# borgwang/tinynn-autograd

Measured on NVIDIA B200. Metric: MLP train samples/sec, higher is better.
Workload: dtype f32 (tensor-core GEMMs: 3-term split on scaled fp16 hi/lo planes, fp32 accumulate)

## Files before the change

### core/_backend.py

```python
import ctypes
import gc
import os
import weakref

import numpy as np

_HERE = os.path.dirname(os.path.abspath(__file__))
_ROOT = os.path.dirname(_HERE)
LIB_PATH = os.environ.get(
    "TNN_B200_LIB", os.path.join(_ROOT, "tinynn-autograd_b200", "libtnn_b200.so"))

F32 = np.dtype(np.float32)
F64 = np.dtype(np.float64)
_DT_CODE = {F32: 0, F64: 1}
MAX_DIMS = 8

ADD, SUB, MUL, DIV, POW, MAXIMUM, MINIMUM, GE, GT, LE, LT, EQ = range(12)
MUL_GE, MUL_GT, MUL_LE, MUL_LT, MUL_EQ, DIV_BWD_B, POW_BWD_A, POW_BWD_B = range(20, 28)
NEG, EXP, LOG, COPY, CLIP, SCALE, CLIP_BWD, RECIP_MUL = range(40, 48)
RED_SUM, RED_MAX, RED_MIN = 0, 1, 2
OPT_SGD, OPT_ADAM, OPT_RMSPROP, OPT_MOMENTUM, OPT_ADAGRAD, OPT_ADADELTA = range(6)

_c_i64 = ctypes.c_int64
_c_i32 = ctypes.c_int32
_c_int = ctypes.c_int
_c_vp = ctypes.c_void_p
_c_dbl = ctypes.c_double
_c_sz = ctypes.c_size_t

_lib = None
_inited = False


class BackendError(RuntimeError):
    pass


_SIGNATURES = {
    "tnn_init": [_c_int],
    "tnn_shutdown": [],
    "tnn_sync": [],
    "tnn_device_info": [_c_vp, _c_vp, _c_vp, _c_vp, _c_vp],
    "tnn_device_count": [_c_vp],
    "tnn_alloc": [_c_sz, _c_vp],
    "tnn_free": [_c_vp],
    "tnn_pool_stats": [_c_vp, _c_vp, _c_vp],
    "tnn_pool_trim": [],
    "tnn_h2d": [_c_vp, _c_vp, _c_sz],
    "tnn_d2h": [_c_vp, _c_vp, _c_sz],
    "tnn_d2d": [_c_vp, _c_vp, _c_sz],
    "tnn_memset": [_c_vp, _c_int, _c_sz],
    "tnn_host_alloc": [_c_sz, _c_vp],
    "tnn_host_free": [_c_vp],
    "tnn_host_register": [_c_vp, _c_sz],
    "tnn_host_unregister": [_c_vp],
    "tnn_h2d_async_copy_stream": [_c_vp, _c_vp, _c_sz],
    "tnn_copy_stream_sync": [],
    "tnn_copy_wait_compute": [],
    "tnn_compute_wait_copy": [],
    "tnn_event_create": [_c_vp],
    "tnn_event_destroy": [_c_vp],
    "tnn_event_record": [_c_vp],
    "tnn_event_elapsed_ms": [_c_vp, _c_vp, _c_vp],
    "tnn_prof_enable": [_c_int],
    "tnn_prof_collect": [_c_vp, _c_vp],
    "tnn_l2_flush": [],
    "tnn_graph_begin": [],
    "tnn_graph_end": [_c_vp],
    "tnn_graph_abort": [],
    "tnn_graph_launch": [_c_vp],
    "tnn_graph_info": [_c_vp, _c_vp, _c_vp, _c_vp],
    "tnn_graph_destroy": [_c_vp],
    "tnn_ew": [_c_int, _c_int, _c_vp, _c_vp, _c_vp, _c_vp, _c_int, _c_vp, _c_vp, _c_vp, _c_vp,
               _c_dbl, _c_dbl, _c_int],
    "tnn_ew_flat": [_c_int, _c_int, _c_vp, _c_vp, _c_vp, _c_vp, _c_i64, _c_int, _c_dbl, _c_dbl,
                    _c_int],
    "tnn_cast": [_c_int, _c_vp, _c_int, _c_vp, _c_i64],
    "tnn_fill": [_c_int, _c_vp, _c_dbl, _c_i64],
    "tnn_reduce": [_c_int, _c_int, _c_vp, _c_vp, _c_i64, _c_i64, _c_i64],
    "tnn_unbroadcast": [_c_int, _c_vp, _c_vp, _c_int, _c_vp, _c_vp],
    "tnn_strided_copy": [_c_int, _c_vp, _c_vp, _c_int, _c_vp, _c_vp, _c_vp],
    "tnn_gather_rows": [_c_int, _c_vp, _c_vp, _c_vp, _c_i64, _c_i64, _c_i64],
    "tnn_scatter_rows": [_c_int, _c_vp, _c_vp, _c_vp, _c_i64, _c_i64, _c_i64],
    "tnn_gather_flat": [_c_int, _c_vp, _c_vp, _c_vp, _c_i64],
    "tnn_scatter_flat": [_c_int, _c_vp, _c_vp, _c_vp, _c_i64],
    "tnn_gemm_simt": [_c_int, _c_vp, _c_i64, _c_vp, _c_i64, _c_i64, _c_vp, _c_i64, _c_i64, _c_i64,
                      _c_i64, _c_i64, _c_vp, _c_int, _c_vp, _c_vp],
    "tnn_dense_bwd_simt": [_c_int, _c_vp, _c_vp, _c_vp, _c_vp, _c_vp, _c_vp, _c_vp, _c_int, _c_vp, _c_int,
                           _c_i64, _c_i64, _c_i64],
    "tnn_split_tf32": [_c_vp, _c_i64, _c_i64, _c_vp, _c_vp, _c_i64, _c_vp, _c_vp, _c_i64],
    "tnn_gemm_tf32x3": [_c_vp, _c_i64, _c_vp, _c_vp, _c_i64, _c_vp, _c_vp, _c_i64, _c_i64, _c_i64,
                        _c_i64, _c_vp, _c_int, _c_int, _c_vp, _c_vp, _c_vp, _c_i64, _c_vp],
    "tnn_split_tf32_bf16": [_c_vp, _c_i64, _c_i64, _c_vp, _c_vp, _c_vp, _c_i64],
    "tnn_gemm_tf32_bf16x2": [_c_vp, _c_i64, _c_vp, _c_vp, _c_vp, _c_i64, _c_vp, _c_vp, _c_vp, _c_i64,
                             _c_i64, _c_i64, _c_i64, _c_vp, _c_int, _c_int, _c_vp, _c_vp, _c_vp, _c_vp,
                             _c_i64, _c_vp],
    "tnn_f16_stats": [_c_vp, _c_i64, _c_vp, _c_int],
    "tnn_set_gemm_f16_cluster": [_c_int],
    "tnn_f16_meta_reset": [_c_vp],
    "tnn_split_f16": [_c_vp, _c_i64, _c_i64, _c_vp, _c_vp, _c_i64, _c_vp, _c_int],
    "tnn_gemm_f16x3": [_c_vp, _c_i64, _c_vp, _c_vp, _c_i64, _c_vp, _c_vp, _c_vp, _c_i64, _c_vp, _c_i64,
                       _c_i64, _c_i64, _c_vp, _c_int, _c_int, _c_vp, _c_vp, _c_vp],
    "tnn_split_tf32_bf16_cond": [_c_vp, _c_i64, _c_i64, _c_vp, _c_vp, _c_vp, _c_i64, _c_int,
                                 _c_vp, _c_i64, _c_i64, _c_vp, _c_vp, _c_vp, _c_i64, _c_int, _c_vp, _c_vp, _c_vp],
    "tnn_f16_stats_cond": [_c_vp, _c_i64, _c_vp, _c_int],
    "tnn_gemm_tf32_bf16x2_cond": [_c_vp, _c_i64, _c_vp, _c_vp, _c_vp, _c_i64, _c_vp, _c_vp, _c_vp, _c_i64,
                                  _c_i64, _c_i64, _c_i64, _c_vp, _c_int, _c_int, _c_vp, _c_vp, _c_vp, _c_vp],
    "tnn_set_gemm_cta_group": [_c_int],
    "tnn_set_gemm_ksplit": [_c_int],
    "tnn_set_gemm_group_m": [_c_int],
    "tnn_relu_fwd": [_c_int, _c_vp, _c_vp, _c_i64],
    "tnn_relu_bwd": [_c_int, _c_vp, _c_vp, _c_vp, _c_i64],
    "tnn_colsum": [_c_int, _c_vp, _c_vp, _c_i64, _c_i64],
    "tnn_ce_stats": [_c_int, _c_vp, _c_i64, _c_i64, _c_vp],
    "tnn_ce_merge_stats": [_c_int, _c_vp, _c_vp, _c_int],
    "tnn_ce_loss": [_c_int, _c_vp, _c_int, _c_vp, _c_i64, _c_i64, _c_vp, _c_dbl, _c_vp, _c_vp, _c_vp],
    "tnn_ce_fwd_small": [_c_int, _c_vp, _c_int, _c_vp, _c_i64, _c_i64, _c_dbl, _c_vp, _c_vp, _c_vp, _c_vp],
    "tnn_ce_bwd": [_c_int, _c_vp, _c_vp, _c_int, _c_vp, _c_i64, _c_i64, _c_vp, _c_vp, _c_dbl, _c_vp, _c_vp,
                   _c_vp],
    "tnn_set_gemm_reserved_sms": [_c_int],
    "tnn_d2h_async": [_c_vp, _c_vp, _c_sz, _c_vp],
    "tnn_event_sync": [_c_vp],
    "tnn_one_hot": [_c_int, _c_vp, _c_vp, _c_i64, _c_i64],
    "tnn_mlp_tail_workspace": [_c_int, _c_vp, _c_vp, _c_i64, _c_vp, _c_vp, _c_vp],
    "tnn_mlp_tail_step": [_c_int, _c_vp, _c_vp, _c_vp, _c_vp, _c_vp, _c_vp, _c_i64, _c_vp, _c_vp, _c_int,
                          _c_i64, _c_dbl, _c_vp, _c_vp, _c_vp, _c_vp, _c_vp, _c_vp, _c_vp],
    "tnn_opt_step": [_c_int, _c_int, _c_vp, _c_vp, _c_vp, _c_vp, _c_vp, _c_i64, _c_vp, _c_int],
    "tnn_opt_step_dev": [_c_int, _c_int, _c_vp, _c_vp, _c_vp, _c_vp, _c_vp, _c_i64, _c_vp],
    "tnn_nccl_unique_id": [_c_vp],
    "tnn_nccl_init": [_c_int, _c_int, _c_vp],
    "tnn_nccl_destroy": [],
    "tnn_allreduce_sum": [_c_int, _c_vp, _c_i64],
    "tnn_allgather": [_c_int, _c_vp, _c_vp, _c_i64],
    "tnn_comm_wait_compute": [],
    "tnn_compute_wait_comm": [],
    "tnn_allreduce_sum_comm": [_c_int, _c_vp, _c_i64],
    "tnn_nccl_version": [_c_vp],
}
EXPORTED_SYMBOLS = sorted(list(_SIGNATURES) + ["tnn_last_error", "tnn_stream", "tnn_launch_count",
                                                "tnn_alloc_ptr"])


def load_library():
    global _lib
    if _lib is not None:
        return _lib
    if not os.path.exists(LIB_PATH):
        raise BackendError(
            "libtnn_b200.so not found at %s -- build it with `python tinynn-autograd_b200/build.py` "
            "(there is no CPU fallback)" % LIB_PATH)
    lib = ctypes.CDLL(LIB_PATH)
    for name, argtypes in _SIGNATURES.items():
        fn = getattr(lib, name)
        fn.argtypes = argtypes
        fn.restype = _c_int
    lib.tnn_last_error.argtypes = []
    lib.tnn_last_error.restype = ctypes.c_char_p
    lib.tnn_stream.argtypes = []
    lib.tnn_stream.restype = _c_vp
    lib.tnn_launch_count.argtypes = []
    lib.tnn_launch_count.restype = ctypes.c_uint64
    lib.tnn_alloc_ptr.argtypes = [_c_sz]
    lib.tnn_alloc_ptr.restype = _c_vp
    _lib = lib
    return lib


def _raise(name):
    msg = _lib.tnn_last_error().decode("utf-8", "replace")
    raise BackendError("%s failed: %s" % (name, msg))


def init(device=None):
    global _inited
    if _inited:
        return
    lib = load_library()
    if device is None:
        device = int(os.environ.get("TNN_DEVICE", os.environ.get("LOCAL_RANK", "0")))
    if lib.tnn_init(int(device)):
        _raise("tnn_init")
    _inited = True


def is_initialized():
    return _inited


def sync():
    init()
    if _lib.tnn_sync():
        _raise("tnn_sync")


def launch_count():
    return int(_lib.tnn_launch_count()) if _lib is not None else 0


def device_info():
    init()
    sm, maj, mnr = _c_int(), _c_int(), _c_int()
    tot, l2 = _c_sz(), _c_sz()
    if _lib.tnn_device_info(ctypes.byref(sm), ctypes.byref(maj), ctypes.byref(mnr),
                            ctypes.byref(tot), ctypes.byref(l2)):
        _raise("tnn_device_info")
    return {"sm_count": sm.value, "cc": (maj.value, mnr.value), "total_mem": tot.value,
            "l2_bytes": l2.value}


def set_gemm_reserved_sms(n):
    init()
    if _lib.tnn_set_gemm_reserved_sms(int(n)):
        _raise("tnn_set_gemm_reserved_sms")


def pool_stats():
    a, b, c = _c_sz(), _c_sz(), _c_sz()
    _lib.tnn_pool_stats(ctypes.byref(a), ctypes.byref(b), ctypes.byref(c))
    return {"reserved": a.value, "in_use": b.value, "cuda_mallocs": c.value}


_SMALL_MAX = 1 << 20
_SMALL_KEEP = 64
_SMALL_CAP_BYTES = 256 << 20
_small_free = {}
_small_bytes = 0
_capturing = False


class _Buf(object):
    __slots__ = ("ptr", "nbytes", "klass", "__weakref__")

    def __init__(self, nbytes):
        self.nbytes = nbytes
        if nbytes <= _SMALL_MAX and not _capturing:
            klass = (nbytes + 511) & ~511
            lst = _small_free.get(klass)
            if lst:
                global _small_bytes
                _small_bytes -= klass
                self.ptr = lst.pop()
                self.klass = klass
                return
            nbytes = klass
            self.klass = klass
        else:
            self.klass = 0
        ptr = _lib.tnn_alloc_ptr(nbytes)
        if not ptr:
            self.ptr = None
            _raise("tnn_alloc")
        self.ptr = ptr

    def __del__(self):
        try:
# ... 184 lines not shown
    arr = np.asarray(arr)
    dt = device_dtype(arr.dtype if dtype is None else dtype)
    host = np.require(arr, dtype=dt, requirements="C")
    out = empty(host.shape, dt)
    if host.size:
        if _lib.tnn_h2d(out.ptr, host.ctypes.data, host.nbytes):
            _raise("tnn_h2d")
    return out


def upload_into(dst, host):
    host = np.require(host, dtype=dst.dtype, requirements="C")
    assert host.size == dst.size
    if host.size and _lib.tnn_h2d(dst.ptr, host.ctypes.data, host.nbytes):
        _raise("tnn_h2d")


def to_numpy(d):
    out = np.empty(d.shape, dtype=d.dtype)
    if d.size:
        if _lib.tnn_d2h(out.ctypes.data, d.ptr, out.nbytes):
            _raise("tnn_d2h")
    return out


def full(shape, value, dtype):
    out = empty(shape, dtype)
    if out.size:
        if _lib.tnn_fill(_DT_CODE[out.dtype], out.ptr, float(value), out.size):
            _raise("tnn_fill")
    return out


_ONES = {}


def ones_scalar(dtype):
    dtype = np.dtype(dtype)
    one = _ONES.get(dtype)
    if one is None:
        one = _ONES[dtype] = full((), 1.0, dtype)
    return one


def zeros(shape, dtype):
    out = empty(shape, dtype)
    if out.size:
        if _lib.tnn_memset(out.ptr, 0, out.nbytes):
            _raise("tnn_memset")
    return out


def memset_zero(d):
    if d.size and _lib.tnn_memset(d.ptr, 0, d.nbytes):
        _raise("tnn_memset")


def copy_into(dst, src):
    assert dst.size == src.size and dst.dtype == src.dtype
    if dst.size and _lib.tnn_d2d(dst.ptr, src.ptr, dst.nbytes):
        _raise("tnn_d2d")


def clone(d):
    out = empty(d.shape, d.dtype)
    copy_into(out, d)
    return out


def astype(d, dtype):
    dtype = np.dtype(dtype)
    if d.dtype == dtype:
        return d
    out = empty(d.shape, dtype)
    if d.size and _lib.tnn_cast(_DT_CODE[dtype], out.ptr, _DT_CODE[d.dtype], d.ptr, d.size):
        _raise("tnn_cast")
    return out


def upload_index(idx):
    idx = np.ascontiguousarray(idx, dtype=np.int64)
    out = empty(idx.shape, F64)
    if idx.size and _lib.tnn_h2d(out.ptr, idx.ctypes.data, idx.nbytes):
        _raise("tnn_h2d")
    return out


def _i64arr(vals):
    return (_c_i64 * len(vals))(*vals)


def _bstrides(shape, out_shape):
    nd = len(out_shape)
    pad = nd - len(shape)
    st = [0] * nd
    acc = 1
    for i in range(len(shape) - 1, -1, -1):
        if shape[i] != 1:
            st[pad + i] = acc
        acc *= shape[i]
    return st


def _common_dtype(*arrs):
    for a in arrs:
        if a.dtype == F64:
            return F64
    return F32


def ew(op, x, y=None, z=None, p0=0.0, p1=0.0, flags=0, out=None):
    ops_ = [a for a in (x, y, z) if a is not None]
    dt = _common_dtype(*ops_)
    ops_ = [a if a.dtype == dt else astype(a, dt) for a in ops_]
    if len(ops_) == 1:
        oshape = ops_[0].shape
    else:
        oshape = ops_[0].shape
        for a in ops_[1:]:
            if a.shape != oshape:
                oshape = np.broadcast_shapes(*[a.shape for a in ops_])
                break
    if out is None:
        out = empty(oshape, dt)
    n = out.size
    if n == 0:
        return out
    ptrs = [a.ptr for a in ops_] + [None] * (3 - len(ops_))
    mask = 0
    flat = True
    for i, a in enumerate(ops_):
        if a.size == 1:
            mask |= 1 << i
        elif a.shape != oshape:
            if a.size == n and _bstrides(a.shape, oshape) == _bstrides(oshape, oshape):
                continue
            flat = False
    if flat:
        if _lib.tnn_ew_flat(op, _DT_CODE[dt], out.ptr, ptrs[0], ptrs[1], ptrs[2], n, mask,
                            p0, p1, flags):
            _raise("tnn_ew_flat")
        return out
    nd = len(oshape)
    if nd > MAX_DIMS:
        raise ValueError("tensors of rank > %d are not supported" % MAX_DIMS)
    st = [_i64arr(_bstrides(a.shape, oshape)) for a in ops_] + [None] * (3 - len(ops_))
    if _lib.tnn_ew(op, _DT_CODE[dt], out.ptr, ptrs[0], ptrs[1], ptrs[2], nd, _i64arr(oshape),
                   st[0], st[1], st[2], p0, p1, flags):
        _raise("tnn_ew")
    return out


def add_inplace(dst, src):
    if src.dtype != dst.dtype:
        src = astype(src, dst.dtype)
    if _lib.tnn_ew_flat(ADD, _DT_CODE[dst.dtype], dst.ptr, dst.ptr, src.ptr, None, dst.size,
                        2 if (src.size == 1 and dst.size != 1) else 0, 0.0, 0.0, 0):
        _raise("tnn_ew_flat")
    return dst


def broadcast_to(d, shape):
    shape = tuple(shape)
    if d.shape == shape:
        return d
    out = empty(shape, d.dtype)
    oshape = np.broadcast_shapes(d.shape, shape)
    if tuple(oshape) != shape:
        raise ValueError("cannot broadcast %s to %s" % (d.shape, shape))
    if out.size:
        if _lib.tnn_ew(COPY, _DT_CODE[d.dtype], out.ptr, d.ptr, None, None, len(shape),
                       _i64arr(shape), _i64arr(_bstrides(d.shape, shape)), None, None, 0.0, 0.0, 0):
            _raise("tnn_ew")
    return out


def reduce(red_op, x, axis=None):
    if axis is None:
        outer, red, inner = 1, x.size, 1
        oshape = ()
    else:
        nd = x.ndim
        if not -nd <= axis < nd:
            raise np.exceptions.AxisError(axis, nd)
        axis %= nd
        outer = _prod(x.shape[:axis])
        red = x.shape[axis]
        inner = _prod(x.shape[axis + 1:])
        oshape = x.shape[:axis] + x.shape[axis + 1:]
    if red == 0 and red_op != RED_SUM:
        raise ValueError("zero-size array to reduction operation which has no identity")
    out = empty(oshape, x.dtype)
    if out.size:
        if _lib.tnn_reduce(red_op, _DT_CODE[x.dtype], out.ptr, x.ptr, outer, red, inner):
            _raise("tnn_reduce")
    return out


def unbroadcast(g, shape):
    shape = tuple(shape)
    if g.shape == shape:
        return g
    nd = g.ndim
    lead = nd - len(shape)
    if lead < 0:
        raise ValueError("gradient of rank %d for a tensor of rank %d" % (nd, len(shape)))
    keep = [0] * lead + [0 if s == 1 else 1 for s in shape]
    for i in range(len(shape)):
        if shape[i] != 1 and shape[i] != g.shape[lead + i]:
            raise ValueError("operands could not be broadcast together with shapes %s %s"
                             % (g.shape, shape))
    out = empty(shape, g.dtype)
    if out.size:
        if _lib.tnn_unbroadcast(_DT_CODE[g.dtype], out.ptr, g.ptr, nd, _i64arr(g.shape),
                                (_c_i32 * nd)(*keep)):
            _raise("tnn_unbroadcast")
    return out


def colsum(g, out=None):
    R, C = g.shape
    if out is None:
        out = empty((1, C), g.dtype)
    if _lib.tnn_colsum(_DT_CODE[g.dtype], out.ptr, g.ptr, R, C):
        _raise("tnn_colsum")
    return out


def _cstrides(shape):
    st = [0] * len(shape)
    acc = 1
    for i in range(len(shape) - 1, -1, -1):
        st[i] = acc
        acc *= shape[i]
    return st


def permute(x, axes):
    nd = x.ndim
    axes = [a % nd for a in axes]
    oshape = tuple(x.shape[a] for a in axes)
    out = empty(oshape, x.dtype)
    if out.size:
        xs = _cstrides(x.shape)
        if _lib.tnn_strided_copy(_DT_CODE[x.dtype], out.ptr, x.ptr, nd, _i64arr(oshape),
                                 _i64arr(_cstrides(oshape)), _i64arr([xs[a] for a in axes])):
            _raise("tnn_strided_copy")
    return out


def strided_copy(dst, dst_off, dst_strides, src, src_off, src_strides, shape):
    if _prod(shape) == 0:
        return
    isz = dst.dtype.itemsize
    if _lib.tnn_strided_copy(_DT_CODE[dst.dtype], dst.ptr + dst_off * isz, src.ptr + src_off * isz,
                             len(shape), _i64arr(shape), _i64arr(dst_strides), _i64arr(src_strides)):
        _raise("tnn_strided_copy")


def one_hot_into(out, labels_i32_ptr, n_rows, n_classes):
    if _lib.tnn_one_hot(_DT_CODE[out.dtype], out.ptr, labels_i32_ptr, n_rows, n_classes):
        _raise("tnn_one_hot")


def gather_rows(x, idx_dev, n_idx):
    row = _prod(x.shape[1:])
    out = empty((n_idx,) + x.shape[1:], x.dtype)
    if out.size and _lib.tnn_gather_rows(_DT_CODE[x.dtype], out.ptr, x.ptr, idx_dev.ptr, n_idx, row,
                                         x.shape[0]):
        _raise("tnn_gather_rows")
    return out


def scatter_rows(g, idx_dev, n_idx, shape):
    out = zeros(shape, g.dtype)
    row = _prod(shape[1:])
    if g.size and _lib.tnn_scatter_rows(_DT_CODE[g.dtype], out.ptr, g.ptr, idx_dev.ptr, n_idx, row,
                                        shape[0]):
        _raise("tnn_scatter_rows")
    return out


def gather_flat(x, idx_dev, oshape):
    out = empty(oshape, x.dtype)
    if out.size and _lib.tnn_gather_flat(_DT_CODE[x.dtype], out.ptr, x.ptr, idx_dev.ptr, out.size):
        _raise("tnn_gather_flat")
    return out


def scatter_flat(g, idx_dev, shape):
    out = zeros(shape, g.dtype)
    if g.size and _lib.tnn_scatter_flat(_DT_CODE[g.dtype], out.ptr, g.ptr, idx_dev.ptr, g.size):
        _raise("tnn_scatter_flat")
    return out


TC_MIN_MNK = int(os.environ.get("TNN_TC_MIN_MNK", str(1 << 29)))
TC_ENABLED = os.environ.get("TNN_TC", "1") != "0"
TC_MN_MAJOR = os.environ.get("TNN_TC_MN_MAJOR", "1") != "0"
TC_SPLIT = os.environ.get("TNN_GEMM_SPLIT", "f16")
LAZY_RELU_OUT = os.environ.get("TNN_LAZY_RELU", "1") != "0"
BF16_BYTES = 2
_split_epoch = 0


def new_split_epoch():
    global _split_epoch
    _split_epoch += 1


def _round4(n):
    return (n + 3) // 4 * 4


def _round8(n):
    return (n + 7) // 8 * 8


def _empty_16bit(rows, ld):
    return empty((rows, ld // 2), F32)


def split_planes_mix(x):
    cache = x.split
    if cache is None or cache.get("epoch") != _split_epoch:
        cache = {"epoch": _split_epoch}
        x.split = cache
    if "m" in cache:
        return cache["m"]
    R, C = x.shape
    ld = _round8(C)
    hi, h16, l16 = empty((R, ld), F32), _empty_16bit(R, ld), _empty_16bit(R, ld)
    if _lib.tnn_split_tf32_bf16(x.ptr, R, C, hi.ptr, h16.ptr, l16.ptr, ld):
        _raise("tnn_split_tf32_bf16")
    cache["m"] = (hi, h16, l16, ld)
    return cache["m"]


F16_PITCH_PAD = int(os.environ.get("TNN_F16_PITCH_PAD", "0"))


def _new_meta():
    return empty((8,), F32)


def split_planes_f16(x):
    cache = x.split
    if cache is None or cache.get("epoch") != _split_epoch:
        cache = {"epoch": _split_epoch}
        x.split = cache
    if "f" in cache:
        return cache["f"]
    R, C = x.shape
    ld = _round8(C) + F16_PITCH_PAD
    if type(x) is LazyReLU and x._real is None:
        src, relu_mode = x._src, 1
    else:
        src, relu_mode = x, 0
    meta = cache.get("stat")
    if meta is None:
        meta = _new_meta()
        if _lib.tnn_f16_stats(src.ptr, R * C, meta.ptr, relu_mode):
            _raise("tnn_f16_stats")
    elif _lib.tnn_f16_stats_cond(src.ptr, R * C, meta.ptr, relu_mode):
        _raise("tnn_f16_stats_cond")
    hf, l16 = _empty_16bit(R, ld), _empty_16bit(R, ld)
    if _lib.tnn_split_f16(src.ptr, R, C, hf.ptr, l16.ptr, ld, meta.ptr, relu_mode):
        _raise("tnn_split_f16")
    cache["f"] = (hf, l16, ld, meta, src if src is not x else None, relu_mode)
    return cache["f"]


_FALLBACK_PLANES = {}
_FALLBACK_CAP_BYTES = 16 << 30
_fallback_bytes = 0


def _fallback_planes(role, R, ld):
    if _capturing:
        return (empty((R, ld), F32), _empty_16bit(R, ld), _empty_16bit(R, ld))
    global _fallback_bytes
    key = (role, R, ld)
    p = _FALLBACK_PLANES.get(key)
    if p is None:
        if _fallback_bytes > _FALLBACK_CAP_BYTES:
            sync()
            _FALLBACK_PLANES.clear()
            _fallback_bytes = 0
        p = (empty((R, ld), F32), _empty_16bit(R, ld), _empty_16bit(R, ld))
        _FALLBACK_PLANES[key] = p
        _fallback_bytes += 8 * R * ld
    return p


def _matmul_f16(a, b, ta, tb, bias, out, flags, act, mask_src, M, N, K):
    a_hf, a_l16, lda, a_meta, a_src, a_relu = split_planes_f16(a)
    b_hf, b_l16, ldb, b_meta, b_src, b_relu = split_planes_f16(b)
    a_src = a if a_src is None else a_src
    b_src = b if b_src is None else b_src
    layout = (1 if ta else 0) | (0 if tb else 2)
    act_out = None
    stat = None
    if act:
        stat = _new_meta()
        if _lib.tnn_f16_meta_reset(stat.ptr):
            _raise("tnn_f16_meta_reset")
        if mask_src is None and LAZY_RELU_OUT:
            act_out = LazyReLU(out)
            flags |= 8
        else:
            act_out = empty((M, N), F32)
    real_act = act_out if (act and type(act_out) is not LazyReLU) else None
    bias_p = bias.ptr if bias is not None else None
    mask_p = mask_src.ptr if (act and mask_src is not None) else None
    if _lib.tnn_gemm_f16x3(out.ptr, N, a_hf.ptr, a_l16.ptr, lda, a_meta.ptr, b_hf.ptr, b_l16.ptr, ldb,
                           b_meta.ptr, M, N, K, bias_p, flags, layout,
                           real_act.ptr if real_act is not None else None, mask_p,
                           stat.ptr if stat is not None else None):
        _raise("tnn_gemm_f16x3")
    fa = _fallback_planes(0, a.shape[0], lda)
    fb = _fallback_planes(1, b.shape[0], ldb)
    if _lib.tnn_split_tf32_bf16_cond(a_src.ptr, a.shape[0], a.shape[1], fa[0].ptr, fa[1].ptr, fa[2].ptr, lda,
                                     a_relu, b_src.ptr, b.shape[0], b.shape[1], fb[0].ptr, fb[1].ptr,
                                     fb[2].ptr, ldb, b_relu, a_meta.ptr, b_meta.ptr,
                                     stat.ptr if stat is not None else None):
        _raise("tnn_split_tf32_bf16_cond")
    if _lib.tnn_gemm_tf32_bf16x2_cond(out.ptr, N, fa[0].ptr, fa[1].ptr, fa[2].ptr, lda, fb[0].ptr, fb[1].ptr,
                                      fb[2].ptr, ldb, M, N, K, bias_p, flags & 3, layout,
                                      real_act.ptr if real_act is not None else None, mask_p,
                                      a_meta.ptr, b_meta.ptr):
        _raise("tnn_gemm_tf32_bf16x2_cond")
    if act:
        act_out.split = {"epoch": _split_epoch, "stat": stat}
        return out, act_out
    return out


def split_planes(x, transposed, also_other=False):
    cache = x.split
    if cache is None or cache.get("epoch") != _split_epoch:
        cache = {"epoch": _split_epoch}
        x.split = cache
    key = "t" if transposed else "p"
    if key in cache:
        return cache[key]
    R, C = x.shape
    want_p = (not transposed) or (also_other and "p" not in cache)
    want_t = transposed or (also_other and "t" not in cache)
    hi = lo = hit = lot = None
    ldp = _round4(C)
    ldt = _round4(R)
    if want_p:
        hi, lo = empty((R, ldp), F32), empty((R, ldp), F32)
    if want_t:
        hit, lot = empty((C, ldt), F32), empty((C, ldt), F32)
    if _lib.tnn_split_tf32(x.ptr, R, C, hi.ptr if hi else None, lo.ptr if lo else None, ldp,
                           hit.ptr if hit else None, lot.ptr if lot else None, ldt):
        _raise("tnn_split_tf32")
    if want_p:
        cache["p"] = (hi, lo, ldp)
    if want_t:
        cache["t"] = (hit, lot, ldt)
    return cache[key]


def set_gemm_cta_group(cg):
    load_library()
    if _lib.tnn_set_gemm_cta_group(int(cg)):
        _raise("tnn_set_gemm_cta_group")


def set_gemm_f16_cluster(cl):
    load_library()
    if _lib.tnn_set_gemm_f16_cluster(int(cl)):
        _raise("tnn_set_gemm_f16_cluster")


def set_gemm_ksplit(ks):
    load_library()
    if _lib.tnn_set_gemm_ksplit(int(ks)):
        _raise("tnn_set_gemm_ksplit")


def use_tensor_cores(M, N, K, dtype):
    return (TC_ENABLED and dtype == F32 and M >= 64 and N >= 64 and K >= 32
            and M * N * K >= TC_MIN_MNK)


def matmul(a, b, ta=False, tb=False, bias=None, out=None, accumulate=False, relu=False,
           reuse_a=False, reuse_b=False, act=False, mask_src=None):
    if a.ndim != 2 or b.ndim != 2:
        raise ValueError("matmul: only 2-D operands are supported (got %s @ %s)" % (a.shape, b.shape))
    dt = _common_dtype(a, b)
    if a.dtype != dt:
        a = astype(a, dt)
    if b.dtype != dt:
        b = astype(b, dt)
    M, K = (a.shape[1], a.shape[0]) if ta else a.shape
    K2, N = (b.shape[1], b.shape[0]) if tb else b.shape
    if K != K2:
        raise ValueError("matmul: shapes %s and %s not aligned" % ((M, K), (K2, N)))
    if out is None:
        out = empty((M, N), dt)
        accumulate = False
    elif out.dtype != dt or out.shape != (M, N):
        raise ValueError("matmul: bad output array")
    if bias is not None and bias.dtype != dt:
        bias = astype(bias, dt)
    act_out = empty((M, N), dt) if act else None
    if M == 0 or N == 0:
        return (out, act_out) if act else out
    flags = (1 if accumulate else 0) | (2 if relu else 0)
    if K > 0 and use_tensor_cores(M, N, K, dt) and TC_SPLIT == "f16":
        return _matmul_f16(a, b, ta, tb, bias, out, flags, act, mask_src, M, N, K)
    if K > 0 and use_tensor_cores(M, N, K, dt) and TC_SPLIT == "mix":
        a_hi, a_h16, a_l16, lda = split_planes_mix(a)
        b_hi, b_h16, b_l16, ldb = split_planes_mix(b)
        layout = (1 if ta else 0) | (0 if tb else 2)
        act_hi = act_h16 = act_l16 = None
        ld_act = _round8(N)
        if act:
            act_hi = empty((M, ld_act), F32)
            act_h16, act_l16 = _empty_16bit(M, ld_act), _empty_16bit(M, ld_act)
            if LAZY_RELU_OUT and mask_src is None:
                act_out = LazyReLU(out)
        if _lib.tnn_gemm_tf32_bf16x2(out.ptr, N, a_hi.ptr, a_h16.ptr, a_l16.ptr, lda, b_hi.ptr,
                                     b_h16.ptr, b_l16.ptr, ldb, M, N, K,
                                     bias.ptr if bias is not None else None, flags, layout,
                                     act_out.ptr if (act and type(act_out) is not LazyReLU) else None,
                                     act_hi.ptr if act else None,
                                     act_h16.ptr if act else None, act_l16.ptr if act else None,
                                     ld_act, mask_src.ptr if (act and mask_src is not None) else None):
            _raise("tnn_gemm_tf32_bf16x2")
        if act:
            act_out.split = {"epoch": _split_epoch, "m": (act_hi, act_h16, act_l16, ld_act)}
            return out, act_out
        return out
    if K > 0 and use_tensor_cores(M, N, K, dt):
        if TC_MN_MAJOR:
            a_hi, a_lo, lda = split_planes(a, transposed=False)
            b_hi, b_lo, ldb = split_planes(b, transposed=False)
            layout = (1 if ta else 0) | (0 if tb else 2)
        else:
            a_hi, a_lo, lda = split_planes(a, transposed=ta, also_other=reuse_a)
            b_hi, b_lo, ldb = split_planes(b, transposed=not tb, also_other=reuse_b)
            layout = 0
        act_hi = act_lo = None
        ld_act = _round4(N)
        if act:
            act_hi, act_lo = empty((M, ld_act), F32), empty((M, ld_act), F32)
        if _lib.tnn_gemm_tf32x3(out.ptr, N, a_hi.ptr, a_lo.ptr, lda, b_hi.ptr, b_lo.ptr, ldb, M, N,
                                K, bias.ptr if bias is not None else None, flags, layout,
                                act_out.ptr if act else None, act_hi.ptr if act else None,
                                act_lo.ptr if act else None, ld_act,
                                mask_src.ptr if (act and mask_src is not None) else None):
            _raise("tnn_gemm_tf32x3")
        if act:
            act_out.split = {"epoch": _split_epoch, "p": (act_hi, act_lo, ld_act)}
            return out, act_out
        return out
    a_rs, a_cs = (1, a.shape[1]) if ta else (a.shape[1], 1)
    b_rs, b_cs = (1, b.shape[1]) if tb else (b.shape[1], 1)
    if mask_src is not None and mask_src.dtype != dt:
        mask_src = astype(mask_src, dt)
    if _lib.tnn_gemm_simt(_DT_CODE[dt], out.ptr, N, a.ptr, a_rs, a_cs, b.ptr, b_rs, b_cs, M, N, K,
                          bias.ptr if bias is not None else None, flags & 1,
                          act_out.ptr if act else None,
                          mask_src.ptr if (act and mask_src is not None) else None):
        _raise("tnn_gemm_simt")
    if relu:
        if _lib.tnn_relu_fwd(_DT_CODE[dt], out.ptr, out.ptr, out.size):
            _raise("tnn_relu_fwd")
    return (out, act_out) if act else out


GROUPED_BWD_MAX_TILES = 1024


def dense_bwd_grouped_ok(B, K, N, dtype):
    if use_tensor_cores(B, K, N, dtype) or use_tensor_cores(K, N, B, dtype):
        return False
    t = lambda m, n: ((m + 31) // 32) * ((n + 31) // 32)
    return t(K, N) + t(B, K) + t(1, N) <= GROUPED_BWD_MAX_TILES


def dense_bwd_grouped(g, x, w, mask_src, need_dx, dw_out, dw_acc, db_out, db_acc):
    B, N = g.shape
    K = w.shape[0]
    dx = empty((B, K), g.dtype) if need_dx else None
    masked = empty((B, K), g.dtype) if (need_dx and mask_src is not None) else None
    if _lib.tnn_dense_bwd_simt(_DT_CODE[g.dtype], g.ptr, x.ptr, w.ptr,
                               mask_src.ptr if masked is not None else None,
                               dx.ptr if dx is not None else None,
                               masked.ptr if masked is not None else None,
                               dw_out.ptr, 1 if dw_acc else 0, db_out.ptr, 1 if db_acc else 0, B, K, N):
        _raise("tnn_dense_bwd_simt")
    return dx, masked


def relu_fwd(x):
    out = empty(x.shape, x.dtype)
    if x.size and _lib.tnn_relu_fwd(_DT_CODE[x.dtype], out.ptr, x.ptr, x.size):
        _raise("tnn_relu_fwd")
    return out


def relu_bwd(g, x):
    if g.dtype != x.dtype:
        g = astype(g, x.dtype)
    out = empty(x.shape, x.dtype)
    if x.size and _lib.tnn_relu_bwd(_DT_CODE[x.dtype], out.ptr, g.ptr, x.ptr, x.size):
        _raise("tnn_relu_bwd")
    return out


def ce_stats(z):
    B, C = z.shape
    stats = empty((2,), z.dtype)
    if _lib.tnn_ce_stats(_DT_CODE[z.dtype], z.ptr, B, C, stats.ptr):
        _raise("tnn_ce_stats")
    return stats


def ce_merge_stats(stats_all, n_ranks):
    out = empty((2,), stats_all.dtype)
    if _lib.tnn_ce_merge_stats(_DT_CODE[stats_all.dtype], out.ptr, stats_all.ptr, n_ranks):
        _raise("tnn_ce_merge_stats")
    return out


def _ce_labels(y):
    if type(y) is LazyOneHot and y._real is None:
        return None, y.labels_ptr
    return y.ptr, None


def ce_loss(z, y, stats, m_global):
    B, C = z.shape
    q = empty((B,), z.dtype)
    loss = empty((), z.dtype)
    y_ptr, lab_ptr = _ce_labels(y)
    if _lib.tnn_ce_loss(_DT_CODE[z.dtype], z.ptr, _DT_CODE[y.dtype], y_ptr, B, C, stats.ptr,
                        float(m_global), q.ptr, loss.ptr, lab_ptr):
        _raise("tnn_ce_loss")
    return loss, q


def ce_small_ok(B, C):
    return B <= 2048 and B * C <= 16384


def ce_fwd_small(z, y, m_global, want_dz=False):
    B, C = z.shape
    stats, q, loss = empty((2,), z.dtype), empty((B,), z.dtype), empty((), z.dtype)
    dz = empty((B, C), z.dtype) if want_dz else None
    if _lib.tnn_ce_fwd_small(_DT_CODE[z.dtype], z.ptr, _DT_CODE[y.dtype], y.ptr, B, C,
                             float(m_global), stats.ptr, q.ptr, loss.ptr, dz.ptr if want_dz else None):
        _raise("tnn_ce_fwd_small")
    return stats, loss, q, dz


def is_ones_scalar(g):
    one = _ONES.get(np.dtype(g.dtype))
    return one is not None and g is one


def ce_bwd(z, y, stats, q, m_global, g):
    B, C = z.shape
    dz = empty((B, C), z.dtype)
    if g.dtype != z.dtype:
        g = astype(g, z.dtype)
    stat = None
    if z.dtype == F32 and TC_SPLIT == "f16" and TC_ENABLED and B * C >= (1 << 16):
        stat = _new_meta()
        if _lib.tnn_f16_meta_reset(stat.ptr):
            _raise("tnn_f16_meta_reset")
    y_ptr, lab_ptr = _ce_labels(y)
    if _lib.tnn_ce_bwd(_DT_CODE[z.dtype], dz.ptr, z.ptr, _DT_CODE[y.dtype], y_ptr, B, C, stats.ptr,
                       q.ptr, float(m_global), g.ptr, stat.ptr if stat is not None else None, lab_ptr):
        _raise("tnn_ce_bwd")
    if stat is not None:
        dz.split = {"epoch": _split_epoch, "stat": stat}
    return dz


class MLPTail(object):

    MAX_WIDTH = 256
    MAX_LAYERS = 6
    SMEM_LIMIT = 220 * 1024

    def __init__(self, dims, batch, n_grad):
        L = len(dims) - 1
        self.L, self.batch, self.n_grad = L, batch, n_grad
        self.in_dims = (_c_i64 * L)(*dims[:-1])
        self.out_dims = (_c_i64 * L)(*dims[1:])
        smem, n_ctas, scratch = _c_i64(), _c_i64(), _c_i64()
        if _lib.tnn_mlp_tail_workspace(L, self.in_dims, self.out_dims, batch, ctypes.byref(smem),
                                       ctypes.byref(n_ctas), ctypes.byref(scratch)):
            _raise("tnn_mlp_tail_workspace")
        self.smem_bytes, self.n_ctas = smem.value, n_ctas.value
        self.scratch = empty((scratch.value,), F32)
        self.stats = zeros((2 * self.n_ctas,), F32)
        self.loss_part = zeros((self.n_ctas,), F32)
        self.counters = zeros((16,), F32)
        self.logits = empty((batch, dims[-1]), F32)
        self.dlogits = self.scratch.view((batch, dims[-1]), scratch.value - batch * dims[-1])

    @classmethod
    def eligible(cls, dims, batch):
        init()
        L = len(dims) - 1
        if not (1 <= L <= cls.MAX_LAYERS) or any(d < 1 or d > cls.MAX_WIDTH for d in dims):
            return False
        if batch < 1 or batch > 256:
            return False
        floats = sum(dims[i] * (dims[i + 1] | 1) + (dims[i + 1] + 3) // 4 * 4 for i in range(L))
        floats = (floats + 3) // 4 * 4 + 12 * sum(dims) + 4 * 256
        return floats * 4 <= cls.SMEM_LIMIT

    def run(self, ws, bs, grad_base, grad_offsets, n_grad, z1, y, m_global, dz1, loss_out):
        if n_grad != self.n_grad:
            raise ValueError("MLPTail was laid out for %d gradient elements, got %d" % (self.n_grad, n_grad))
        wp = (_c_vp * self.L)(*[w.ptr for w in ws])
        bp = (_c_vp * self.L)(*[b.ptr for b in bs])
        go = (_c_i64 * (2 * self.L))(*grad_offsets)
        if _lib.tnn_mlp_tail_step(self.L, self.in_dims, self.out_dims, wp, bp, go, grad_base.ptr, n_grad,
                                  z1.ptr, y.ptr, _DT_CODE[y.dtype], self.batch, float(m_global), dz1.ptr,
                                  loss_out.ptr, self.scratch.ptr, self.stats.ptr, self.loss_part.ptr,
                                  self.counters.ptr, self.logits.ptr):
            _raise("tnn_mlp_tail_step")


def opt_step(opt, param, step_out, grad, s0, s1, hyper):
    n = grad.size
    if isinstance(hyper, DArray):
        if _lib.tnn_opt_step_dev(opt, _DT_CODE[grad.dtype], param.ptr if param is not None else None,
                                 step_out.ptr if step_out is not None else None, grad.ptr,
                                 s0.ptr if s0 is not None else None,
                                 s1.ptr if s1 is not None else None, n, hyper.ptr):
            _raise("tnn_opt_step_dev")
        return
    h = (_c_dbl * len(hyper))(*hyper)
    if _lib.tnn_opt_step(opt, _DT_CODE[grad.dtype], param.ptr if param is not None else None,
                         step_out.ptr if step_out is not None else None, grad.ptr,
                         s0.ptr if s0 is not None else None, s1.ptr if s1 is not None else None,
                         n, h, len(hyper)):
        _raise("tnn_opt_step")


class PinnedArray(object):

    def __init__(self, shape, dtype):
        init()
        self.shape = tuple(shape)
        self.dtype = np.dtype(dtype)
        nbytes = max(_prod(self.shape), 1) * self.dtype.itemsize
        p = _c_vp()
        if _lib.tnn_host_alloc(nbytes, ctypes.byref(p)):
            _raise("tnn_host_alloc")
        self.ptr = p.value
        self.nbytes = nbytes
        raw = (ctypes.c_char * nbytes).from_address(self.ptr)
        self.array = np.frombuffer(raw, dtype=self.dtype, count=_prod(self.shape)).reshape(self.shape)

    def __del__(self):
        try:
            if self.ptr and _lib is not None:
                self.array = None
                _lib.tnn_host_free(self.ptr)
                self.ptr = None
        except Exception:
            pass


class RegisteredHostArray(object):

    def __init__(self, array):
        init()
        if not (isinstance(array, np.ndarray) and array.flags["C_CONTIGUOUS"]):
            raise ValueError("only C-contiguous numpy arrays can be pinned in place")
        self.array = array
        self.ptr = array.ctypes.data
        if _lib.tnn_host_register(self.ptr, array.nbytes):
            _raise("tnn_host_register")

    def row_address(self, row):
        return self.ptr + row * self.array.strides[0]

    def __del__(self):
        try:
            if self.ptr and _lib is not None:
                _lib.tnn_host_unregister(self.ptr)
                self.ptr = None
        except Exception:
            pass


def h2d_prefetch(dst, pinned):
    if _lib.tnn_copy_wait_compute():
        _raise("tnn_copy_wait_compute")
    src = pinned if isinstance(pinned, int) else pinned.ptr
    if _lib.tnn_h2d_async_copy_stream(dst.ptr, src, dst.nbytes):
        _raise("tnn_h2d_async_copy_stream")


def copy_stream_sync():
    if _lib.tnn_copy_stream_sync():
        _raise("tnn_copy_stream_sync")


def wait_prefetch():
    if _lib.tnn_compute_wait_copy():
        _raise("tnn_compute_wait_copy")


_pinned_free = {}


class AsyncRead(object):

    def __init__(self, d):
        init()
        self.shape, self.dtype = d.shape, d.dtype
        nbytes = max(d.nbytes, 1)
        free = _pinned_free.get(nbytes)
        self.pin = free.pop() if free else PinnedArray((nbytes,), np.uint8)
        self.event = Event()
        self._src = d
        self._value = None
        if _lib.tnn_d2h_async(self.pin.ptr, d.ptr, d.nbytes, self.event.ptr):
            _raise("tnn_d2h_async")

    def result(self):
        if self._value is None:
# ... 130 lines not shown
```

### include/tnn_b200.h

```cpp
#ifndef TNN_B200_H
#define TNN_B200_H

#include <stddef.h>
#include <stdint.h>

#ifdef __cplusplus
extern "C" {
#endif

#define TNN_MAX_DIMS 8
#define TNN_F32 0
#define TNN_F64 1

enum {
  TNN_OP_ADD = 0,
  TNN_OP_SUB = 1,
  TNN_OP_MUL = 2,
  TNN_OP_DIV = 3,
  TNN_OP_POW = 4,
  TNN_OP_MAXIMUM = 5,
  TNN_OP_MINIMUM = 6,
  TNN_OP_GE = 7,
  TNN_OP_GT = 8,
  TNN_OP_LE = 9,
  TNN_OP_LT = 10,
  TNN_OP_EQ = 11,
  TNN_OP_MUL_GE = 20,
  TNN_OP_MUL_GT = 21,
  TNN_OP_MUL_LE = 22,
  TNN_OP_MUL_LT = 23,
  TNN_OP_MUL_EQ = 24,
  TNN_OP_DIV_BWD_B = 25,
  TNN_OP_POW_BWD_A = 26,
  TNN_OP_POW_BWD_B = 27,
  TNN_OP_NEG = 40,
  TNN_OP_EXP = 41,
  TNN_OP_LOG = 42,
  TNN_OP_COPY = 43,
  TNN_OP_CLIP = 44,
  TNN_OP_SCALE = 45,
  TNN_OP_CLIP_BWD = 46,
  TNN_OP_RECIP_MUL = 47
};

enum { TNN_RED_SUM = 0, TNN_RED_MAX = 1, TNN_RED_MIN = 2 };

enum {
  TNN_OPT_SGD = 0,
  TNN_OPT_ADAM = 1,
  TNN_OPT_RMSPROP = 2,
  TNN_OPT_MOMENTUM = 3,
  TNN_OPT_ADAGRAD = 4,
  TNN_OPT_ADADELTA = 5
};

const char* tnn_last_error(void);
int tnn_init(int device);
int tnn_shutdown(void);
int tnn_sync(void);
int tnn_device_info(int* sm_count, int* cc_major, int* cc_minor, size_t* total_mem, size_t* l2_bytes);
int tnn_device_count(int* n);
void* tnn_stream(void);
uint64_t tnn_launch_count(void);

int tnn_alloc(size_t nbytes, void** out);
void* tnn_alloc_ptr(size_t nbytes);
int tnn_free(void* p);
int tnn_pool_stats(size_t* reserved_bytes, size_t* in_use_bytes, size_t* n_cuda_malloc);
int tnn_pool_trim(void);
int tnn_h2d(void* dst, const void* src, size_t nbytes);
int tnn_d2h(void* dst, const void* src, size_t nbytes);
int tnn_d2h_async(void* pinned_dst, const void* src, size_t nbytes, void* done_event);
int tnn_event_sync(void* ev);
int tnn_d2d(void* dst, const void* src, size_t nbytes);
int tnn_memset(void* dst, int byte, size_t nbytes);
int tnn_host_alloc(size_t nbytes, void** out);
int tnn_host_free(void* p);
int tnn_host_register(void* p, size_t nbytes);
int tnn_host_unregister(void* p);
int tnn_h2d_async_copy_stream(void* dst, const void* pinned_src, size_t nbytes);
int tnn_copy_stream_sync(void);
int tnn_copy_wait_compute(void);
int tnn_compute_wait_copy(void);
int tnn_event_create(void** ev);
int tnn_event_destroy(void* ev);
int tnn_event_record(void* ev);
int tnn_event_elapsed_ms(void* start, void* stop, float* ms);
int tnn_prof_enable(int family);
int tnn_prof_collect(double* total_ms, uint64_t* n_launches);
int tnn_l2_flush(void);

int tnn_graph_begin(void);
int tnn_graph_end(void** graph_out);
int tnn_graph_abort(void);
int tnn_graph_launch(void* graph);
int tnn_graph_info(void* graph, size_t* n_nodes, size_t* n_kernel_nodes, size_t* n_blocks);
int tnn_graph_destroy(void* graph);

int tnn_ew(int op, int dtype, void* out, const void* x, const void* y, const void* z,
           int ndim, const int64_t* shape,
           const int64_t* xs, const int64_t* ys, const int64_t* zs,
           double p0, double p1, int flags);
int tnn_ew_flat(int op, int dtype, void* out, const void* x, const void* y, const void* z,
                int64_t n, int scalar_mask, double p0, double p1, int flags);
int tnn_cast(int dst_dtype, void* dst, int src_dtype, const void* src, int64_t n);
int tnn_fill(int dtype, void* dst, double value, int64_t n);

int tnn_reduce(int red_op, int dtype, void* out, const void* x,
               int64_t outer, int64_t red, int64_t inner);
int tnn_unbroadcast(int dtype, void* out, const void* grad, int ndim,
                    const int64_t* gshape, const int32_t* keep);

int tnn_strided_copy(int dtype, void* dst, const void* src, int ndim, const int64_t* shape,
                     const int64_t* dst_strides, const int64_t* src_strides);
int tnn_gather_rows(int dtype, void* out, const void* x, const int64_t* idx_dev,
                    int64_t n_idx, int64_t row_elems, int64_t n_rows_src);
int tnn_scatter_rows(int dtype, void* out, const void* g, const int64_t* idx_dev,
                     int64_t n_idx, int64_t row_elems, int64_t n_rows_dst);
int tnn_gather_flat(int dtype, void* out, const void* x, const int64_t* idx_dev, int64_t n);
int tnn_scatter_flat(int dtype, void* out, const void* g, const int64_t* idx_dev, int64_t n);
int tnn_one_hot(int dtype, void* out, const int32_t* labels_dev, int64_t B, int64_t C);

int tnn_gemm_simt(int dtype, void* C, int64_t ldc, const void* A, int64_t a_rs, int64_t a_cs,
                  const void* B, int64_t b_rs, int64_t b_cs, int64_t M, int64_t N, int64_t K,
                  const void* bias, int flags, void* act_out, const void* mask_src);
int tnn_dense_bwd_simt(int dtype, const void* g, const void* x, const void* w, const void* mask_src,
                       void* dx, void* dx_masked, void* dw, int dw_accumulate, void* db,
                       int db_accumulate, int64_t B, int64_t K, int64_t N);
int tnn_split_tf32(const float* x, int64_t R, int64_t C,
                   float* hi, float* lo, int64_t ldp, float* hiT, float* loT, int64_t ldt);
int tnn_gemm_tf32x3(float* D, int64_t ldd,
                    const float* a_hi, const float* a_lo, int64_t lda,
                    const float* b_hi, const float* b_lo, int64_t ldb,
                    int64_t M, int64_t N, int64_t K, const float* bias, int flags, int layout,
                    float* act_out, float* act_hi, float* act_lo, int64_t ld_act,
                    const float* mask_src);
int tnn_split_tf32_bf16(const float* x, int64_t R, int64_t C, float* hi, void* h16, void* l16,
                        int64_t ld);
int tnn_gemm_tf32_bf16x2(float* D, int64_t ldd,
                         const float* a_hi, const void* a_h16, const void* a_l16, int64_t lda,
                         const float* b_hi, const void* b_h16, const void* b_l16, int64_t ldb,
                         int64_t M, int64_t N, int64_t K, const float* bias, int flags, int layout,
                         float* act_out, float* act_hi, void* act_h16, void* act_l16, int64_t ld_act,
                         const float* mask_src);
int tnn_f16_stats(const float* x, int64_t n, void* meta, int relu_mode);
int tnn_set_gemm_f16_cluster(int cl);
int tnn_f16_meta_reset(void* meta);
int tnn_split_f16(const float* x, int64_t R, int64_t C, void* hf, void* l16, int64_t ld, void* meta,
                  int relu_mode);
int tnn_gemm_f16x3(float* D, int64_t ldd, const void* a_hf, const void* a_l16, int64_t lda,
                   const void* a_meta, const void* b_hf, const void* b_l16, int64_t ldb,
                   const void* b_meta, int64_t M, int64_t N, int64_t K, const float* bias, int flags,
                   int layout, float* act_out, const float* mask_src, void* stat_meta);
int tnn_split_tf32_bf16_cond(const float* xa, int64_t Ra, int64_t Ca, float* hia, void* h16a, void* l16a,
                             int64_t lda, int relu_a, const float* xb, int64_t Rb, int64_t Cb, float* hib,
                             void* h16b, void* l16b, int64_t ldb, int relu_b, const void* meta_a,
                             const void* meta_b, void* result_meta);
int tnn_f16_stats_cond(const float* x, int64_t n, void* meta, int relu_mode);
int tnn_gemm_tf32_bf16x2_cond(float* D, int64_t ldd, const float* a_hi, const void* a_h16,
                              const void* a_l16, int64_t lda, const float* b_hi, const void* b_h16,
                              const void* b_l16, int64_t ldb, int64_t M, int64_t N, int64_t K,
                              const float* bias, int flags, int layout, float* act_out,
                              const float* mask_src, const void* meta_a, const void* meta_b);
int tnn_set_gemm_cta_group(int cg);
int tnn_set_gemm_reserved_sms(int n);
int tnn_set_gemm_ksplit(int ks);
int tnn_set_gemm_group_m(int gm);

int tnn_relu_fwd(int dtype, void* out, const void* x, int64_t n);
int tnn_relu_bwd(int dtype, void* dx, const void* g, const void* x, int64_t n);
int tnn_colsum(int dtype, void* out, const void* g, int64_t R, int64_t C);

int tnn_ce_stats(int dtype, const void* z, int64_t B, int64_t C, void* stats_dev);
int tnn_ce_merge_stats(int dtype, void* stats_out_dev, const void* stats_all_dev, int n_ranks);
int tnn_ce_loss(int dtype, const void* z, int y_dtype, const void* y, int64_t B, int64_t C,
                const void* stats_dev, double m_global, void* q_dev, void* loss_dev,
                const int32_t* labels_dev);
int tnn_ce_fwd_small(int dtype, const void* z, int y_dtype, const void* y, int64_t B, int64_t C,
                     double m_global, void* stats_dev, void* q_dev, void* loss_dev,
                     void* dz_dev );
int tnn_ce_bwd(int dtype, void* dz, const void* z, int y_dtype, const void* y, int64_t B, int64_t C,
               const void* stats_dev, const void* q_dev, double m_global, const void* g_dev,
               void* stat_meta ,
               const int32_t* labels_dev);

int tnn_mlp_tail_workspace(int n_layers, const int64_t* in_dims, const int64_t* out_dims, int64_t batch,
                           int64_t* smem_bytes, int64_t* n_ctas, int64_t* scratch_floats);
int tnn_mlp_tail_step(int n_layers, const int64_t* in_dims, const int64_t* out_dims, const void* const* w,
                      const void* const* b, const int64_t* grad_off, void* grad, int64_t n_grad,
                      const void* z1, const void* y, int y_dtype, int64_t B, double m_global, void* dz1,
                      void* loss_out, void* scratch, void* stats, void* loss_part, void* counters,
                      void* logits_out );

int tnn_opt_step(int opt, int dtype, void* param, void* step_out, const void* grad, void* s0,
                 void* s1, int64_t n, const double* h, int n_h);
int tnn_opt_step_dev(int opt, int dtype, void* param, void* step_out, const void* grad, void* s0,
                     void* s1, int64_t n, const double* h_dev);

int tnn_nccl_unique_id(void* id128);
int tnn_nccl_init(int rank, int world, const void* id128);
int tnn_nccl_destroy(void);
int tnn_allreduce_sum(int dtype, void* buf, int64_t n);
int tnn_allgather(int dtype, void* recv, const void* send, int64_t n_per_rank);
int tnn_comm_wait_compute(void);
int tnn_compute_wait_comm(void);
int tnn_allreduce_sum_comm(int dtype, void* buf, int64_t n);
int tnn_nccl_version(int* v);

#ifdef __cplusplus
}
#endif
#endif
```

### tinynn-autograd_b200/build.py

```python
import concurrent.futures
import os
import shutil
import subprocess
import sys

HERE = os.path.dirname(os.path.abspath(__file__))
ROOT = os.path.dirname(HERE)
CSRC = os.path.join(HERE, "csrc")
OBJ = os.path.join(HERE, "build")
LIB = os.path.join(HERE, "libtnn_b200.so")

SOURCES = ["runtime.cu", "elementwise.cu", "reduce.cu", "layout.cu", "gemm_simt.cu",
           "gemm_tc.cu", "gemm_f16.cu", "fused.cu", "mlp_fused.cu", "comm.cu"]
HEADERS = [os.path.join(CSRC, "common.cuh"), os.path.join(CSRC, "math.cuh"), os.path.join(CSRC, "tc_ptx.cuh"),
           os.path.join(ROOT, "include", "tnn_b200.h")]

NVCC_FLAGS = ["-gencode", "arch=compute_100a,code=sm_100a", "-O3", "-lineinfo", "-std=c++17",
              "-Xcompiler", "-fPIC", "-diag-suppress", "550", "-split-compile", "0"]
NO_FMAD = {"elementwise.cu", "fused.cu", "reduce.cu"}


def _nvcc():
    return shutil.which("nvcc") or "/usr/local/cuda/bin/nvcc"


def _stale(target, deps):
    if not os.path.exists(target):
        return True
    t = os.path.getmtime(target)
    return any(os.path.getmtime(d) > t for d in deps)


def _compile(src, force):
    obj = os.path.join(OBJ, src.replace(".cu", ".o"))
    path = os.path.join(CSRC, src)
    if not force and not _stale(obj, [path] + HEADERS):
        return obj, False
    cmd = [_nvcc()] + NVCC_FLAGS + (["-fmad=false"] if src in NO_FMAD else []) + ["-c", path, "-o", obj]
    r = subprocess.run(cmd, capture_output=True, text=True)
    if r.returncode != 0:
        raise RuntimeError("nvcc failed for %s:\n%s\n%s" % (src, r.stdout[-4000:], r.stderr[-4000:]))
    return obj, True


def build(force=False, verbose=True):
    os.makedirs(OBJ, exist_ok=True)
    with concurrent.futures.ThreadPoolExecutor(max_workers=min(8, len(SOURCES))) as ex:
        results = list(ex.map(lambda s: _compile(s, force), SOURCES))
    objs = [o for o, _ in results]
    rebuilt = any(changed for _, changed in results)
    if rebuilt or _stale(LIB, objs):
        cmd = [_nvcc(), "-shared", "-o", LIB] + objs + ["-ldl"]
        r = subprocess.run(cmd, capture_output=True, text=True)
        if r.returncode != 0:
            raise RuntimeError("link failed:\n%s\n%s" % (r.stdout[-4000:], r.stderr[-4000:]))
        if verbose:
            print("built", LIB)
    elif verbose:
        print("up to date:", LIB)
    return LIB


if __name__ == "__main__":
    build(force="--force" in sys.argv)
```

### tinynn-autograd_b200/csrc/gemm_f16.cu

```cuda
#include <cuda.h>
#include <cuda_bf16.h>
#include <cuda_fp16.h>
#include <cudaTypedefs.h>

#include <algorithm>
#include <cstdlib>

#include "common.cuh"
#include "tc_ptx.cuh"

namespace tnn {
namespace tc {
extern int g_reserved_sms;
}
namespace f16 {

using namespace tnn::tc;

#ifndef TNN_F16_BK
#define TNN_F16_BK 64
#endif
#ifndef TNN_F16_STAGES
#define TNN_F16_STAGES (192 / TNN_F16_BK)
#endif
constexpr int BK = TNN_F16_BK;
constexpr int ROWS = 128;
constexpr int UMMA_N = 256;
constexpr int TILE_M = 256;
constexpr int UMMA_K = 16;
constexpr int PLANE_BYTES = ROWS * BK * 2;
constexpr int STAGE_BYTES = 4 * PLANE_BYTES;
constexpr int STAGES = TNN_F16_STAGES;
constexpr int CHUNK_KB = 256 / BK;
#ifndef TNN_F16_THREADS
#define TNN_F16_THREADS 384
#endif
constexpr int NUM_THREADS = TNN_F16_THREADS;
constexpr int EPI_WARP0 = NUM_THREADS == 320 ? 2 : 4;
constexpr uint32_t TMEM_COLS = 512;
constexpr int EPI_PATCH_BYTES = 8 * 4096;
constexpr int SMEM_BYTES = STAGES * STAGE_BYTES + 1024 + 256 + EPI_PATCH_BYTES;
#ifndef TNN_F16_KBOX_ROWS
#define TNN_F16_KBOX_ROWS 128
#endif
constexpr int KBOX_ROWS = TNN_F16_KBOX_ROWS;
constexpr int MN_BOX_BYTES = 64 * BK * 2;
constexpr float SMALL_LIMIT = 0.03125f;
constexpr unsigned int GUARD_FRACTION = 256;

struct Meta {
  unsigned int absmax;
  unsigned int need_stats;
  int exp;
  int safe;
  unsigned int n_small;
  unsigned int n_nz;
  unsigned int ticket;
  unsigned int pad;
};

__device__ __forceinline__ void meta_scale(unsigned int amax_bits, int& e, int& ok) {
  e = 0;
  ok = 1;
  if (amax_bits == 0u) return;
  if (amax_bits >= 0x7F800000u) { ok = 0; return; }
  const int ex = (int)(amax_bits >> 23) - 127;
  if (ex < -112) { ok = 0; return; }
  e = 14 - ex;
}

__device__ __forceinline__ float pow2f(int e) {
  return __int_as_float((e + 127) << 23);
}

template <bool MN>
__device__ __forceinline__ uint64_t make_desc(uint32_t saddr) {
  uint64_t d = 0;
  d |= (uint64_t)((saddr & 0x3FFFFu) >> 4);
  d |= (uint64_t)(MN ? (MN_BOX_BYTES >> 4) : 1) << 16;
  d |= (uint64_t)(((MN || BK == 64) ? 1024 : 512) >> 4) << 32;
  d |= (uint64_t)1 << 46;
  d |= (uint64_t)((MN || BK == 64) ? 2 : 4) << 61;
  return d;
}
__host__ __device__ constexpr uint32_t make_idesc(int a_fmt, int b_fmt, bool a_mn, bool b_mn) {
  return (1u << 4) | ((uint32_t)a_fmt << 7) | ((uint32_t)b_fmt << 10) | ((a_mn ? 1u : 0u) << 15) |
         ((b_mn ? 1u : 0u) << 16) | ((uint32_t)(UMMA_N >> 3) << 17) | ((uint32_t)(TILE_M >> 4) << 24);
}

__device__ __forceinline__ void tile_coords(int t, int tiles_m, int tiles_n, int group_m, int& tm, int& tn) {
  if (group_m == 1) {
    tm = t / tiles_n;
    tn = t - tm * tiles_n;
  } else if (group_m < 0) {
    const int gn = -group_m;
    const int per_panel = tiles_m * gn;
    const int g = t / per_panel;
    const int first_n = g * gn;
    const int cols = min(gn, tiles_n - first_n);
    const int r = t - g * per_panel;
    tm = r / cols;
    tn = first_n + r % cols;
  } else {
    const int per_group = group_m * tiles_n;
    const int g = t / per_group;
    const int first_m = g * group_m;
    const int rows = min(group_m, tiles_m - first_m);
    const int r = t - g * per_group;
    tm = first_m + r % rows;
    tn = r / rows;
  }
}

template <int CB>
__device__ __forceinline__ void patch_write(const float (&sum)[128], float4* patch, int lane, float f1,
                                            float f2, const float* bias_u, int colb, int N) {
#pragma unroll
  for (int c4 = 0; c4 < 8; ++c4) {
    float4 v = make_float4(sum[CB * 32 + c4 * 4] * f1 * f2, sum[CB * 32 + c4 * 4 + 1] * f1 * f2,
                           sum[CB * 32 + c4 * 4 + 2] * f1 * f2, sum[CB * 32 + c4 * 4 + 3] * f1 * f2);
    if (bias_u) {
      const int c = colb + c4 * 4;
      if (c + 3 < N) {
        const float4 b = *reinterpret_cast<const float4*>(bias_u + c);
        v.x += b.x; v.y += b.y; v.z += b.z; v.w += b.w;
      } else {
        if (c < N) v.x += bias_u[c];
        if (c + 1 < N) v.y += bias_u[c + 1];
        if (c + 2 < N) v.z += bias_u[c + 2];
      }
    }
    patch[lane * 8 + (c4 ^ (lane & 7))] = v;
  }
}

template <bool A_MN, bool B_MN, int CL>
__global__ void __launch_bounds__(NUM_THREADS, 1)
gemm_f16x3_kernel(const __grid_constant__ CUtensorMap map_a_h, const __grid_constant__ CUtensorMap map_a_l,
                  const __grid_constant__ CUtensorMap map_b_h, const __grid_constant__ CUtensorMap map_b_l,
                  float* __restrict__ D, int64_t ldd, int M, int N, int K,
                  const float* __restrict__ bias, int flags, int t_full, int tail_split,
                  unsigned int* __restrict__ tile_flags, float* __restrict__ act_out,
                  const float* __restrict__ mask_src, const Meta* __restrict__ meta_a,
                  const Meta* __restrict__ meta_b, Meta* __restrict__ stat_out, int group_m) {
  if (!(meta_a->safe && meta_b->safe)) return;
  extern __shared__ uint8_t smem_raw[];
  const uint32_t smem_base = (smem_u32(smem_raw) + 1023u) & ~1023u;
  uint8_t* smem_gen = smem_raw + (smem_base - smem_u32(smem_raw));
  const uint32_t bar_base = smem_base + STAGES * STAGE_BYTES;
  auto full_bar = [&](int s) { return bar_base + 8u * s; };
  auto empty_bar = [&](int s) { return bar_base + 8u * (STAGES + s); };
  auto tfull_bar = [&](int a) { return bar_base + 8u * (2 * STAGES + a); };
  auto tempty_bar = [&](int a) { return bar_base + 8u * (2 * STAGES + 2 + a); };
  const uint32_t tmem_ptr_smem = bar_base + 8u * (2 * STAGES + 4);
  volatile uint32_t* tmem_ptr_gen =
      reinterpret_cast<volatile uint32_t*>(smem_gen + STAGES * STAGE_BYTES + 8 * (2 * STAGES + 4));

  const int warp = threadIdx.x >> 5, lane = threadIdx.x & 31;
  const uint32_t cl_rank = cluster_ctarank();
  const uint32_t pair = cl_rank >> 1;
  const uint32_t cta_rank = cl_rank & 1u;
  const bool leader = cta_rank == 0;
  const uint16_t pair_mask = (uint16_t)(3u << (2 * pair));

  if (warp == 0 && lane == 0) {
    tma_prefetch_desc(&map_a_h);
    tma_prefetch_desc(&map_a_l);
    tma_prefetch_desc(&map_b_h);
    tma_prefetch_desc(&map_b_l);
    for (int s = 0; s < STAGES; ++s) {
      mbar_init(full_bar(s), 1);
      mbar_init(empty_bar(s), CL / 2);
    }
    for (int a = 0; a < 2; ++a) {
      mbar_init(tfull_bar(a), 1);
      mbar_init(tempty_bar(a), 16);
    }
    fence_barrier_init();
  }
  if (warp == 1) {
    tmem_alloc<2>(tmem_ptr_smem, TMEM_COLS);
    tmem_relinquish<2>();
  }
  tc_fence_before();
  cluster_sync_all();
  tc_fence_after();
  const uint32_t tmem_base = *tmem_ptr_gen;

  const int tiles_m = (M + TILE_M - 1) / TILE_M;
  const int tiles_n = (N + UMMA_N - 1) / UMMA_N;
  const int tiles_ns = CL == 4 ? (tiles_n + 1) / 2 : tiles_n;
  const int num_tiles = tiles_m * tiles_ns;
  const int num_kb = (K + BK - 1) / BK;
  const int group = blockIdx.x / CL;
  const int num_groups = gridDim.x / CL;
  const int tail_rem = num_tiles - t_full;
  const int num_units = t_full + tail_rem * tail_split;
  const int kb_per_split = (num_kb + tail_split - 1) / tail_split;
  auto decode = [&](int u, int& t, int& sp, int& kb_begin, int& kb_end) {
    if (u < t_full) {
      t = u; sp = 0; kb_begin = 0; kb_end = num_kb;
    } else {
      const int j = u - t_full;
      t = t_full + j % tail_rem;
      sp = j / tail_rem;
      kb_begin = sp * kb_per_split;
      kb_end = min(num_kb, kb_begin + kb_per_split);
    }
  };

  if (warp == 0) {
    if constexpr (NUM_THREADS == 384) asm volatile("setmaxnreg.dec.sync.aligned.u32 40;");
    if (lane == 0) {
      int stage = 0;
      uint32_t phase = 0;
      for (int u = group; u < num_units; u += num_groups) {
        int t, sp, kb_begin, kb_end;
        decode(u, t, sp, kb_begin, kb_end);
        int tm, tn;
        tile_coords((flags & 32) ? num_tiles - 1 - t : t, tiles_m, tiles_ns, group_m, tm, tn);
        if constexpr (CL == 4) tn = 2 * tn + (int)pair;
        const int row_a = tm * TILE_M + (int)cta_rank * ROWS;
        const int row_b = tn * UMMA_N + (int)cta_rank * ROWS;
        for (int kb = kb_begin; kb < kb_end; ++kb) {
          mbar_wait(empty_bar(stage), phase ^ 1u);
          const uint32_t sa_h = smem_base + stage * STAGE_BYTES;
          const uint32_t sa_l = sa_h + PLANE_BYTES;
          const uint32_t sb_h = sa_h + 2 * PLANE_BYTES;
          const uint32_t sb_l = sa_h + 3 * PLANE_BYTES;
          if (leader) mbar_expect_tx(full_bar(stage), (uint32_t)STAGE_BYTES * 2u);
          const int k0 = kb * BK;
          if (flags & 128) {
            if (leader)
              asm volatile("mbarrier.complete_tx.shared::cta.b64 [%0], %1;" ::"r"(full_bar(stage)), "r"((uint32_t)STAGE_BYTES * 2u) : "memory");
            if (++stage == STAGES) { stage = 0; phase ^= 1u; }
            continue;
          }
#ifdef TNN_F16_PREFETCH
          if (kb + TNN_F16_PREFETCH < kb_end) {
            const int kp = (kb + TNN_F16_PREFETCH) * BK;
            if constexpr (A_MN) {
#pragma unroll
              for (int j = 0; j < ROWS / 64; ++j) {
                tma_prefetch_l2_2d(&map_a_l, row_a + 64 * j, kp);
                tma_prefetch_l2_2d(&map_a_h, row_a + 64 * j, kp);
              }
            } else {
              tma_prefetch_l2_2d(&map_a_l, kp, row_a);
              tma_prefetch_l2_2d(&map_a_h, kp, row_a);
            }
            if constexpr (B_MN) {
#pragma unroll
              for (int j = 0; j < ROWS / 64; ++j) {
                tma_prefetch_l2_2d(&map_b_h, row_b + 64 * j, kp);
                tma_prefetch_l2_2d(&map_b_l, row_b + 64 * j, kp);
              }
            } else {
              tma_prefetch_l2_2d(&map_b_h, kp, row_b);
              tma_prefetch_l2_2d(&map_b_l, kp, row_b);
            }
          }
#endif
          if constexpr (CL == 4) {
            const uint16_t mc = (uint16_t)((1u << cta_rank) | (1u << (cta_rank + 2)));
            const uint32_t off = pair * (uint32_t)(PLANE_BYTES / 2);
            const int ra = row_a + 64 * (int)pair;
            if constexpr (A_MN) {
              tma_load_2d_pair_mc(sa_l + off, &map_a_l, full_bar(stage), ra, k0, mc);
              tma_load_2d_pair_mc(sa_h + off, &map_a_h, full_bar(stage), ra, k0, mc);
            } else {
              tma_load_2d_pair_mc(sa_l + off, &map_a_l, full_bar(stage), k0, ra, mc);
              tma_load_2d_pair_mc(sa_h + off, &map_a_h, full_bar(stage), k0, ra, mc);
            }
          } else if constexpr (A_MN) {
#pragma unroll
            for (int j = 0; j < ROWS / 64; ++j) {
              tma_load_2d<2>(sa_l + j * MN_BOX_BYTES, &map_a_l, full_bar(stage), row_a + 64 * j, k0);
              tma_load_2d<2>(sa_h + j * MN_BOX_BYTES, &map_a_h, full_bar(stage), row_a + 64 * j, k0);
            }
          } else {
#pragma unroll
            for (int j = 0; j < ROWS / KBOX_ROWS; ++j) {
              tma_load_2d<2>(sa_l + j * KBOX_ROWS * 128, &map_a_l, full_bar(stage), k0, row_a + j * KBOX_ROWS);
              tma_load_2d<2>(sa_h + j * KBOX_ROWS * 128, &map_a_h, full_bar(stage), k0, row_a + j * KBOX_ROWS);
            }
          }
          if constexpr (B_MN) {
#pragma unroll
            for (int j = 0; j < ROWS / 64; ++j) {
              tma_load_2d<2>(sb_h + j * MN_BOX_BYTES, &map_b_h, full_bar(stage), row_b + 64 * j, k0);
              tma_load_2d<2>(sb_l + j * MN_BOX_BYTES, &map_b_l, full_bar(stage), row_b + 64 * j, k0);
            }
          } else {
#pragma unroll
            for (int j = 0; j < ROWS / KBOX_ROWS; ++j) {
              tma_load_2d<2>(sb_h + j * KBOX_ROWS * 128, &map_b_h, full_bar(stage), k0, row_b + j * KBOX_ROWS);
              tma_load_2d<2>(sb_l + j * KBOX_ROWS * 128, &map_b_l, full_bar(stage), k0, row_b + j * KBOX_ROWS);
            }
// ... 193 lines not shown
                    v.z = fmaxf(v.z, 0.f); v.w = fmaxf(v.w, 0.f);
                  }
                  *reinterpret_cast<float4*>(dp) = v;
                  if (want_relu_side) {
                    v.x = v.x < 0.f ? 0.f : v.x; v.y = v.y < 0.f ? 0.f : v.y;
                    v.z = v.z < 0.f ? 0.f : v.z; v.w = v.w < 0.f ? 0.f : v.w;
                    if (emit_act) *reinterpret_cast<float4*>(ap) = v;
                  }
                  if (want_stats)
                    st_max = max(max(st_max, __float_as_uint(v.x) & 0x7FFFFFFFu),
                                 max(max(__float_as_uint(v.y) & 0x7FFFFFFFu, __float_as_uint(v.z) & 0x7FFFFFFFu),
                                     __float_as_uint(v.w) & 0x7FFFFFFFu));
                }
                dp += step;
                if (emit_act) ap += step;
              }
            } else {
              const int nrows = min(32, M - row_base);
              const float4* pp0 = patch + rr * 8 + (c4l ^ rr);
              const float4* pp1 = patch + (rr + 4) * 8 + (c4l ^ (rr + 4));
              const int64_t off0 = (int64_t)(row_base + rr) * ldd + gcol, step = 4 * ldd;
              float4 pre[8];
              {
                const float* sp_ = pre_src + off0;
#pragma unroll
                for (int i = 0; i < 8; ++i) {
                  if (4 * i + rr < nrows) pre[i] = *reinterpret_cast<const float4*>(sp_);
                  sp_ += step;
                }
              }
              float* dp = D + off0;
              float* ap = emit_act ? act_out + off0 : nullptr;
              const float* mp = (want_mask && accumulate) ? mask_src + off0 : nullptr;
#pragma unroll
              for (int i = 0; i < 8; ++i) {
                if (4 * i + rr < nrows) {
                  float4 v = (i & 1) ? pp1[(i >> 1) * 64] : pp0[(i >> 1) * 64];
                  if (accumulate) {
                    v.x += pre[i].x; v.y += pre[i].y; v.z += pre[i].z; v.w += pre[i].w;
                  }
                  if (relu) {
                    v.x = fmaxf(v.x, 0.f); v.y = fmaxf(v.y, 0.f);
                    v.z = fmaxf(v.z, 0.f); v.w = fmaxf(v.w, 0.f);
                  }
                  *reinterpret_cast<float4*>(dp) = v;
                  if (want_mask) {
                    const float4 z = accumulate ? *reinterpret_cast<const float4*>(mp) : pre[i];
                    v.x = z.x >= 0.f ? v.x : v.x * 0.f; v.y = z.y >= 0.f ? v.y : v.y * 0.f;
                    v.z = z.z >= 0.f ? v.z : v.z * 0.f; v.w = z.w >= 0.f ? v.w : v.w * 0.f;
                  } else if (want_relu_side) {
                    v.x = v.x < 0.f ? 0.f : v.x; v.y = v.y < 0.f ? 0.f : v.y;
                    v.z = v.z < 0.f ? 0.f : v.z; v.w = v.w < 0.f ? 0.f : v.w;
                  }
                  if (emit_act) *reinterpret_cast<float4*>(ap) = v;
                  if (want_stats)
                    st_max = max(max(st_max, __float_as_uint(v.x) & 0x7FFFFFFFu),
                                 max(max(__float_as_uint(v.y) & 0x7FFFFFFFu, __float_as_uint(v.z) & 0x7FFFFFFFu),
                                     __float_as_uint(v.w) & 0x7FFFFFFFu));
                }
                dp += step;
                if (emit_act) ap += step;
                if (mp) mp += step;
              }
            }
          } else {
#pragma unroll 1
            for (int i = 0; i < 8; ++i) {
              const int r = 4 * i + rr, grow = row_base + r;
              if (grow >= M) break;
              const float4 v4 = patch[r * 8 + (c4l ^ (r & 7))];
              const float s[4] = {v4.x, v4.y, v4.z, v4.w};
#pragma unroll 1
              for (int k = 0; k < 4; ++k) {
                if (gcol + k >= N) break;
                const int64_t off = (int64_t)grow * ldd + gcol + k;
                float x = k == 0 ? s[0] : (k == 1 ? s[1] : (k == 2 ? s[2] : s[3]));
                if (accumulate) x += D[off];
                if (relu) x = fmaxf(x, 0.f);
                D[off] = x;
                float a = x;
                if (want_mask) a = mask_src[off] >= 0.f ? x : x * 0.f;
                else if (want_relu_side) a = x < 0.f ? 0.f : x;
                if (emit_act) act_out[off] = a;
                if (want_stats) st_max = max(st_max, __float_as_uint(a) & 0x7FFFFFFFu);
              }
            }
          }
          __syncwarp();
        }
      }
#ifdef TNN_F16_PROBE
      ep_store += clock64() - q1;
#endif
      if (u >= t_full && sp + 1 < tail_split && tile_valid) {
        __threadfence();
        __syncwarp();
        if (lane == 0) atomicAdd(tile_flags + flag_idx, 1u);
      }
    }
#ifdef TNN_F16_PROBE
    if ((group == 0 || group == 37) && warp == 4 && lane == 0 && cta_rank == 0)
      printf("probe group %d epilogue warp 4: total %lld cycles, waiting for a chunk %lld, storing tiles %lld\n",
             group, clock64() - ep_begin, ep_wait, ep_store);
#endif
    if (stat_out != nullptr) {
      st_max = __reduce_max_sync(0xFFFFFFFFu, st_max);
      if (lane == 0 && st_max) atomicMax(&stat_out->absmax, st_max);
    }
  }

  __syncwarp();
  tc_fence_before();
  cluster_sync_all();
  if (warp == 1) {
    tc_fence_after();
    tmem_dealloc<2>(tmem_base, TMEM_COLS);
  }
}


__global__ void __launch_bounds__(256)
stats_kernel(const float* __restrict__ x, int64_t n, Meta* __restrict__ meta, int relu_mode, int vec,
             int only_if_needed) {
  if (only_if_needed && !meta->need_stats) return;
  unsigned int mx = 0u;
  const int64_t stride = (int64_t)gridDim.x * blockDim.x;
  auto take = [&](float v) {
    if (relu_mode && v < 0.f) v = 0.f;
    mx = max(mx, __float_as_uint(v) & 0x7FFFFFFFu);
  };
  if (vec) {
    const int64_t n4 = n / 4;
    const float4* x4 = reinterpret_cast<const float4*>(x);
    for (int64_t i = (int64_t)blockIdx.x * blockDim.x + threadIdx.x; i < n4; i += stride) {
      const float4 t = x4[i];
      take(t.x); take(t.y); take(t.z); take(t.w);
    }
    for (int64_t i = n4 * 4 + (int64_t)blockIdx.x * blockDim.x + threadIdx.x; i < n; i += stride) take(x[i]);
  } else {
    for (int64_t i = (int64_t)blockIdx.x * blockDim.x + threadIdx.x; i < n; i += stride) take(x[i]);
  }
  mx = __reduce_max_sync(0xFFFFFFFFu, mx);
  __shared__ unsigned int s_mx[8];
  const int warp = threadIdx.x >> 5, lane = threadIdx.x & 31;
  if (lane == 0) s_mx[warp] = mx;
  __syncthreads();
  if (threadIdx.x == 0) {
#pragma unroll
    for (int w = 1; w < 8; ++w) mx = max(mx, s_mx[w]);
    if (mx) atomicMax(&meta->absmax, mx);
  }
}

__global__ void __launch_bounds__(256)
split_f16_kernel(const float* __restrict__ x, int64_t R, int64_t C, __half* __restrict__ hf,
                 __half* __restrict__ l16, int64_t ld, Meta* __restrict__ meta, int relu_mode,
                 int vec_in) {
  int e, ok;
  meta_scale(meta->absmax, e, ok);
  const float sc = ok ? pow2f(e) : 1.f;
  const int64_t gpr = ld / 8;
  const int64_t total = R * gpr;
  const int64_t stride = (int64_t)gridDim.x * blockDim.x;
  unsigned int n_small = 0u, n_nz = 0u;
  if (ok) {
    for (int64_t i = (int64_t)blockIdx.x * blockDim.x + threadIdx.x; i < total; i += stride) {
      const int64_t r = i / gpr, c = (i - r * gpr) * 8;
      float v[8];
      if (vec_in && c + 7 < C) {
        const float4 t0 = *reinterpret_cast<const float4*>(x + r * C + c);
        const float4 t1 = *reinterpret_cast<const float4*>(x + r * C + c + 4);
        v[0] = t0.x; v[1] = t0.y; v[2] = t0.z; v[3] = t0.w;
        v[4] = t1.x; v[5] = t1.y; v[6] = t1.z; v[7] = t1.w;
      } else {
#pragma unroll
        for (int k = 0; k < 8; ++k) v[k] = (c + k < C) ? x[r * C + c + k] : 0.f;
      }
      union { __half2 h[4]; uint4 u; } ph, pl;
#pragma unroll
      for (int k = 0; k < 4; ++k) {
        float a = v[2 * k], b = v[2 * k + 1];
        if (relu_mode) { a = a < 0.f ? 0.f : a; b = b < 0.f ? 0.f : b; }
        a *= sc; b *= sc;
        n_nz += (a != 0.f) + (b != 0.f);
        n_small += (a != 0.f && fabsf(a) < SMALL_LIMIT) + (b != 0.f && fabsf(b) < SMALL_LIMIT);
        const __half2 h = __floats2half2_rn(a, b);
        const float2 hb = __half22float2(h);
        ph.h[k] = h;
        pl.h[k] = __floats2half2_rn(a - hb.x, b - hb.y);
      }
      *reinterpret_cast<uint4*>(hf + r * ld + c) = ph.u;
      *reinterpret_cast<uint4*>(l16 + r * ld + c) = pl.u;
    }
  }
  n_small = __reduce_add_sync(0xFFFFFFFFu, n_small);
  n_nz = __reduce_add_sync(0xFFFFFFFFu, n_nz);
  __shared__ unsigned int s_small[8], s_nz[8];
  const int warp = threadIdx.x >> 5, lane = threadIdx.x & 31;
  if (lane == 0) { s_small[warp] = n_small; s_nz[warp] = n_nz; }
  __syncthreads();
  if (threadIdx.x == 0) {
#pragma unroll
    for (int w = 1; w < 8; ++w) { n_small += s_small[w]; n_nz += s_nz[w]; }
    if (n_small) atomicAdd(&meta->n_small, n_small);
    if (n_nz) atomicAdd(&meta->n_nz, n_nz);
    __threadfence();
    if (atomicAdd(&meta->ticket, 1u) == gridDim.x - 1) {
      __threadfence();
      const unsigned int ts = *reinterpret_cast<volatile unsigned int*>(&meta->n_small);
      const unsigned int tn = *reinterpret_cast<volatile unsigned int*>(&meta->n_nz);
      meta->exp = e;
      meta->safe = (ok && (unsigned long long)ts * GUARD_FRACTION <= (unsigned long long)tn) ? 1 : 0;
    }
  }
}

static PFN_cuTensorMapEncodeTiled_v12000 g_encode = nullptr;

static int get_encode_fn() {
  if (g_encode) return 0;
  void* fn = nullptr;
  cudaDriverEntryPointQueryResult qres;
  TNN_CUDA(cudaGetDriverEntryPointByVersion("cuTensorMapEncodeTiled", &fn, 12000, cudaEnableDefault, &qres));
  if (qres != cudaDriverEntryPointSuccess || !fn) TNN_FAIL("cuTensorMapEncodeTiled is not available");
  g_encode = (PFN_cuTensorMapEncodeTiled_v12000)fn;
  return 0;
}

static int make_map(CUtensorMap* map, const void* ptr, int64_t rows, int64_t K, int64_t ld,
                    bool mn_major, int box_rows = ROWS) {
  if ((reinterpret_cast<uintptr_t>(ptr) & 15) != 0) TNN_FAIL("f16 GEMM: operand plane must be 16-byte aligned");
  if (ld % 8 != 0) TNN_FAIL("f16 GEMM: operand pitch must be a multiple of 8 elements");
  cuuint64_t dims[2] = {(cuuint64_t)(mn_major ? rows : K), (cuuint64_t)(mn_major ? K : rows)};
  cuuint64_t strides[1] = {(cuuint64_t)ld * 2};
  cuuint32_t box[2] = {(cuuint32_t)(mn_major ? 64 : BK), (cuuint32_t)(mn_major ? BK : box_rows)};
  cuuint32_t estr[2] = {1, 1};
  CUresult r = g_encode(map, CU_TENSOR_MAP_DATA_TYPE_FLOAT16, 2,
                        (void*)ptr, dims, strides, box, estr, CU_TENSOR_MAP_INTERLEAVE_NONE,
                        (mn_major || BK == 64) ? CU_TENSOR_MAP_SWIZZLE_128B : CU_TENSOR_MAP_SWIZZLE_64B,
                        CU_TENSOR_MAP_L2_PROMOTION_L2_256B,
                        CU_TENSOR_MAP_FLOAT_OOB_FILL_NONE);
  if (r != CUDA_SUCCESS) TNN_FAIL("cuTensorMapEncodeTiled (f16 planes) failed with code " + std::to_string((int)r));
  return 0;
}

static unsigned int* g_tile_flags = nullptr;
constexpr int MAX_FLAG_TILES = 1 << 16;
static bool g_attr_set[2][2][2] = {};
static int g_group_m = -8;
static bool g_reverse = true;
static int g_cluster = 2;

template <bool A_MN, bool B_MN, int CL>
static int launch(float* D, int64_t ldd, const void* a_h, const void* a_l, int64_t lda, const void* b_h,
                  const void* b_l, int64_t ldb, int64_t M, int64_t N, int64_t K, const float* bias,
                  int flags, float* act_out, const float* mask_src, const Meta* meta_a,
                  const Meta* meta_b, Meta* stat_out) {
  CUtensorMap ma_h, ma_l, mb_h, mb_l;
  if (make_map(&ma_h, a_h, M, K, lda, A_MN, CL == 4 ? 64 : KBOX_ROWS)) return 1;
  if (make_map(&ma_l, a_l, M, K, lda, A_MN, CL == 4 ? 64 : KBOX_ROWS)) return 1;
  if (make_map(&mb_h, b_h, N, K, ldb, B_MN, KBOX_ROWS)) return 1;
  if (make_map(&mb_l, b_l, N, K, ldb, B_MN, KBOX_ROWS)) return 1;
  auto kern = gemm_f16x3_kernel<A_MN, B_MN, CL>;
  if (!g_attr_set[A_MN][B_MN][CL == 4]) {
    TNN_CUDA(cudaFuncSetAttribute(kern, cudaFuncAttributeMaxDynamicSharedMemorySize, SMEM_BYTES));
    g_attr_set[A_MN][B_MN][CL == 4] = true;
  }
  const int64_t tiles_m = ceil_div(M, TILE_M), tiles_n = ceil_div(N, UMMA_N);
  const int64_t tiles = tiles_m * (CL == 4 ? ceil_div(tiles_n, 2) : tiles_n);
  const int max_groups = std::max(1, (ctx().sm_count - tc::g_reserved_sms) / CL);
  int t_full = (int)tiles, tail_split = 1;
  if (!(flags & 2) && tiles_m * tiles_n <= MAX_FLAG_TILES) {
    const int64_t num_kb = ceil_div(K, BK);
    const int64_t rem = tiles % max_groups;
    if (rem > 0) {
      int s = 1;
      while (s < 4 && rem * (s * 2) <= max_groups && num_kb / (s * 2) >= 512 / BK) s *= 2;
      if (s > 1) {
        t_full = (int)(tiles - rem);
        tail_split = s;
      }
    }
  }
  if (tail_split > 1) {
    if (!g_tile_flags) TNN_CUDA(cudaMalloc(&g_tile_flags, MAX_FLAG_TILES * sizeof(unsigned int)));
    TNN_CUDA(cudaMemsetAsync(g_tile_flags, 0, (size_t)(tiles_m * tiles_n) * sizeof(unsigned int), ctx().stream));
  }
  const int64_t units = t_full + (tiles - t_full) * tail_split;
  const int groups = (int)std::min<int64_t>(units, max_groups);
  cudaLaunchConfig_t cfg = {};
  cfg.gridDim = dim3((unsigned)(groups * CL));
  cfg.blockDim = dim3(NUM_THREADS);
  cfg.dynamicSmemBytes = SMEM_BYTES;
  cfg.stream = ctx().stream;
  cudaLaunchAttribute attr[1];
  attr[0].id = cudaLaunchAttributeClusterDimension;
  attr[0].val.clusterDim.x = CL;
  attr[0].val.clusterDim.y = 1;
  attr[0].val.clusterDim.z = 1;
  cfg.attrs = attr;
  cfg.numAttrs = 1;
  if constexpr (CL == 4) {
    static int max_clusters = 0;
    if (!max_clusters) {
      TNN_CUDA(cudaOccupancyMaxActiveClusters(&max_clusters, kern, &cfg));
      if (max_clusters < 1) max_clusters = 1;
    }
    if (groups > max_clusters) cfg.gridDim = dim3((unsigned)(max_clusters * CL));
  }
  const int gm = (CL == 4 && g_group_m < 0) ? std::min(-1, g_group_m / 2) : g_group_m;
  prof_begin(1);
  TNN_CUDA(cudaLaunchKernelEx(&cfg, kern, ma_h, ma_l, mb_h, mb_l, D, ldd, (int)M, (int)N, (int)K, bias, flags,
                              t_full, tail_split, g_tile_flags, act_out, mask_src, meta_a, meta_b, stat_out, gm));
  ctx().launches++;
  prof_end(1);
  return 0;
}

template <int CL>
static int launch_layout(int layout, float* D, int64_t ldd, const void* a_h, const void* a_l, int64_t lda,
                         const void* b_h, const void* b_l, int64_t ldb, int64_t M, int64_t N, int64_t K,
                         const float* bias, int flags, float* act_out, const float* mask_src,
                         const Meta* ma, const Meta* mb, Meta* st) {
  switch (layout & 3) {
    case 0: return launch<false, false, CL>(D, ldd, a_h, a_l, lda, b_h, b_l, ldb, M, N, K, bias, flags, act_out, mask_src, ma, mb, st);
    case 1: return launch<true, false, CL>(D, ldd, a_h, a_l, lda, b_h, b_l, ldb, M, N, K, bias, flags, act_out, mask_src, ma, mb, st);
    case 2: return launch<false, true, CL>(D, ldd, a_h, a_l, lda, b_h, b_l, ldb, M, N, K, bias, flags, act_out, mask_src, ma, mb, st);
    default: return launch<true, true, CL>(D, ldd, a_h, a_l, lda, b_h, b_l, ldb, M, N, K, bias, flags, act_out, mask_src, ma, mb, st);
  }
}

}
}

using namespace tnn;

extern "C" {

int tnn_set_gemm_f16_cluster(int cl) {
  if (cl != 2 && cl != 4) TNN_FAIL("tnn_set_gemm_f16_cluster: 2 (CTA pairs) or 4 (two pairs sharing A by TMA multicast)");
  f16::g_cluster = cl;
  return 0;
}

int tnn_f16_stats(const float* x, int64_t n, void* meta, int relu_mode) {
  TNN_REQUIRE_INIT();
  if (!meta) TNN_FAIL("tnn_f16_stats: meta is required");
  TNN_CUDA(cudaMemsetAsync(meta, 0, sizeof(f16::Meta), ctx().stream));
  if (n <= 0) return 0;
  const int vec = (reinterpret_cast<uintptr_t>(x) & 15) == 0;
  prof_begin(3);
  f16::stats_kernel<<<ew_grid(ceil_div(n, 16), 256), 256, 0, ctx().stream>>>(x, n, (f16::Meta*)meta, relu_mode, vec, 0);
  TNN_POST_LAUNCH();
  prof_end(3);
  return 0;
}

int tnn_f16_stats_cond(const float* x, int64_t n, void* meta, int relu_mode) {
  TNN_REQUIRE_INIT();
  if (!meta) TNN_FAIL("tnn_f16_stats_cond: meta is required");
  if (n <= 0) return 0;
  const int vec = (reinterpret_cast<uintptr_t>(x) & 15) == 0;
  prof_begin(3);
  f16::stats_kernel<<<ew_grid(ceil_div(n, 16), 256, 4), 256, 0, ctx().stream>>>(x, n, (f16::Meta*)meta, relu_mode, vec, 1);
  TNN_POST_LAUNCH();
  prof_end(3);
  return 0;
}

int tnn_f16_meta_reset(void* meta) {
  TNN_REQUIRE_INIT();
  if (!meta) TNN_FAIL("tnn_f16_meta_reset: meta is required");
  TNN_CUDA(cudaMemsetAsync(meta, 0, sizeof(f16::Meta), ctx().stream));
  return 0;
}

int tnn_split_f16(const float* x, int64_t R, int64_t C, void* hf, void* l16, int64_t ld, void* meta,
                  int relu_mode) {
  TNN_REQUIRE_INIT();
  if (R <= 0 || C <= 0) return 0;
  if (!hf || !l16 || !meta) TNN_FAIL("tnn_split_f16: both planes and the meta record are required");
  if (ld % 8 != 0 || ld < C) TNN_FAIL("tnn_split_f16: ld must be >= C and a multiple of 8");
  const int vec_in = (C % 4 == 0) && ((reinterpret_cast<uintptr_t>(x) & 15) == 0);
  prof_begin(3);
  f16::split_f16_kernel<<<ew_grid(R * (ld / 8), 256), 256, 0, ctx().stream>>>(
      x, R, C, (__half*)hf, (__half*)l16, ld, (f16::Meta*)meta, relu_mode, vec_in);
  TNN_POST_LAUNCH();
  prof_end(3);
  return 0;
}

int tnn_gemm_f16x3(float* D, int64_t ldd, const void* a_hf, const void* a_l16, int64_t lda,
                   const void* a_meta, const void* b_hf, const void* b_l16, int64_t ldb,
                   const void* b_meta, int64_t M, int64_t N, int64_t K, const float* bias, int flags,
                   int layout, float* act_out, const float* mask_src, void* stat_meta) {
  TNN_REQUIRE_INIT();
  if (M <= 0 || N <= 0) return 0;
  if (K <= 0) TNN_FAIL("tnn_gemm_f16x3: K must be positive");
  if (M > 2147483647LL || N > 2147483647LL || K > 2147483647LL) TNN_FAIL("tnn_gemm_f16x3: extent above int32");
  if (!a_meta || !b_meta) TNN_FAIL("tnn_gemm_f16x3: operand meta records are required");
  if (mask_src && !act_out) TNN_FAIL("tnn_gemm_f16x3: the mask_src form needs act_out");
  if (act_out && (flags & 2)) TNN_FAIL("tnn_gemm_f16x3: act_out and the relu-in-place flag are exclusive");
  if (f16::get_encode_fn()) return 1;
  if (getenv("TNN_EXP_FLAGS")) flags |= atoi(getenv("TNN_EXP_FLAGS")) & (128 | 256);
  static bool env_read = false;
  if (!env_read) {
    const char* gm = getenv("TNN_F16_GROUP_M");
    if (gm && atoi(gm) != 0 && atoi(gm) >= -64 && atoi(gm) <= 64) f16::g_group_m = atoi(gm);
    const char* rv = getenv("TNN_F16_REVERSE");
    if (rv) f16::g_reverse = atoi(rv) != 0;
    const char* cl = getenv("TNN_F16_CLUSTER");
    if (cl && (atoi(cl) == 2 || atoi(cl) == 4)) f16::g_cluster = atoi(cl);
    env_read = true;
  }
  if (f16::g_reverse) flags |= 32;
  const f16::Meta* ma = (const f16::Meta*)a_meta;
  const f16::Meta* mb = (const f16::Meta*)b_meta;
  f16::Meta* st = (f16::Meta*)stat_meta;
  if (f16::g_cluster == 4 && N > f16::UMMA_N)
    return f16::launch_layout<4>(layout, D, ldd, a_hf, a_l16, lda, b_hf, b_l16, ldb, M, N, K, bias, flags, act_out, mask_src, ma, mb, st);
  return f16::launch_layout<2>(layout, D, ldd, a_hf, a_l16, lda, b_hf, b_l16, ldb, M, N, K, bias, flags, act_out, mask_src, ma, mb, st);
}

}
```

### tinynn-autograd_b200/csrc/gemm_tc.cu

```cuda
#include <cuda.h>
#include <cuda_bf16.h>
#include <cudaTypedefs.h>

#include <algorithm>
#include <cstdlib>

#include "common.cuh"

namespace tnn {
namespace tc {

constexpr int BK = 32;
constexpr int ROWS_A = 128;
constexpr int UMMA_N = 256;
constexpr int UMMA_K = 8;
constexpr int PLANE_ROW_BYTES = BK * 4;
constexpr int NUM_THREADS = 384;
#ifndef TNN_CHUNK_KB
#define TNN_CHUNK_KB 8
#endif
constexpr int CHUNK_KB = TNN_CHUNK_KB;
constexpr uint32_t TMEM_COLS = 512;

template <int CG>
// ... 491 lines not shown
                if (accumulate) {
                  const float4 o = pre[i];
                  v.x += o.x; v.y += o.y; v.z += o.z; v.w += o.w;
                }
                if (relu) {
                  v.x = fmaxf(v.x, 0.f); v.y = fmaxf(v.y, 0.f);
                  v.z = fmaxf(v.z, 0.f); v.w = fmaxf(v.w, 0.f);
                }
                *reinterpret_cast<float4*>(dp) = v;
                if (emit_act) {
                  float4 a;
                  if (mask_src) {
                    const float4 z = accumulate
                        ? *reinterpret_cast<const float4*>(mask_src + (int64_t)grow * ldd + gcol)
                        : pre[i];
                    a = make_float4(z.x >= 0.f ? v.x : v.x * 0.f, z.y >= 0.f ? v.y : v.y * 0.f,
                                    z.z >= 0.f ? v.z : v.z * 0.f, z.w >= 0.f ? v.w : v.w * 0.f);
                  } else {
                    a = make_float4(v.x < 0.f ? 0.f : v.x, v.y < 0.f ? 0.f : v.y,
                                    v.z < 0.f ? 0.f : v.z, v.w < 0.f ? 0.f : v.w);
                  }
                  if (act_out) *reinterpret_cast<float4*>(act_out + (int64_t)grow * ldd + gcol) = a;
                  if (act_hi) {
                    const float4 h = make_float4(to_tf32(a.x), to_tf32(a.y), to_tf32(a.z), to_tf32(a.w));
                    *reinterpret_cast<float4*>(act_hi + (int64_t)grow * ld_act + gcol) = h;
                    if constexpr (!MIX) {
                      const float4 l = make_float4(to_tf32(a.x - h.x), to_tf32(a.y - h.y),
                                                   to_tf32(a.z - h.z), to_tf32(a.w - h.w));
                      *reinterpret_cast<float4*>(act_lo + (int64_t)grow * ld_act + gcol) = l;
                    } else {
                      __nv_bfloat16* h16p = reinterpret_cast<__nv_bfloat16*>(act_lo);
                      union { __nv_bfloat162 b[2]; uint2 u; } ph, pl;
                      ph.b[0] = __floats2bfloat162_rn(a.x, a.y);
                      ph.b[1] = __floats2bfloat162_rn(a.z, a.w);
                      pl.b[0] = __floats2bfloat162_rn(a.x - h.x, a.y - h.y);
                      pl.b[1] = __floats2bfloat162_rn(a.z - h.z, a.w - h.w);
                      *reinterpret_cast<uint2*>(h16p + (int64_t)grow * ld_act + gcol) = ph.u;
                      *reinterpret_cast<uint2*>(act_l16 + (int64_t)grow * ld_act + gcol) = pl.u;
                    }
                  }
                }
              } else {
                const float e[4] = {v.x, v.y, v.z, v.w};
#pragma unroll
                for (int k = 0; k < 4; ++k) {
                  if (gcol + k < N) {
                    float x = e[k];
                    if (accumulate) x += dp[k];
                    if (relu) x = fmaxf(x, 0.f);
                    dp[k] = x;
                    if (emit_act) {
                      float a;
                      if (mask_src) a = mask_src[(int64_t)grow * ldd + gcol + k] >= 0.f ? x : x * 0.f;
                      else a = x < 0.f ? 0.f : x;
                      if (act_out) act_out[(int64_t)grow * ldd + gcol + k] = a;
                      if (act_hi) {
                        const float h = to_tf32(a);
                        act_hi[(int64_t)grow * ld_act + gcol + k] = h;
                        if constexpr (!MIX) {
                          act_lo[(int64_t)grow * ld_act + gcol + k] = to_tf32(a - h);
                        } else {
                          reinterpret_cast<__nv_bfloat16*>(act_lo)[(int64_t)grow * ld_act + gcol + k] =
                              __float2bfloat16_rn(a);
                          act_l16[(int64_t)grow * ld_act + gcol + k] = __float2bfloat16_rn(a - h);
                        }
                      }
                    }
                  }
                }
              }
            }
          }
          __syncwarp();
        }
      }
      if (u >= t_full && sp + 1 < tail_split) {
        __threadfence();
        __syncwarp();
        if (lane == 0) atomicAdd(tile_flags + t, 1u);
      }
    }
  }

  __syncwarp();
  tc_fence_before();
  if constexpr (CG == 1) __syncthreads();
  else cluster_sync_all();
  if (warp == 1) {
    tc_fence_after();
    tmem_dealloc<CG>(tmem_base, TMEM_COLS);
  }
}


__global__ void __launch_bounds__(256)
split_tf32_kernel(const float* __restrict__ x, int64_t R, int64_t C, float* __restrict__ hi,
                  float* __restrict__ lo, int64_t ldp, float* __restrict__ hiT,
                  float* __restrict__ loT, int64_t ldt, int vec_in) {
  __shared__ float tile[64][65];
  const int64_t r0 = (int64_t)blockIdx.y * 64, c0 = (int64_t)blockIdx.x * 64;
  const int tx = threadIdx.x & 15, ty = threadIdx.x >> 4;
#pragma unroll
  for (int i = 0; i < 4; ++i) {
    const int lr = ty + 16 * i;
    const int64_t r = r0 + lr, c = c0 + tx * 4;
    float v[4] = {0.f, 0.f, 0.f, 0.f};
    if (r < R) {
      if (vec_in && c + 3 < C) {
        const float4 t = *reinterpret_cast<const float4*>(x + r * C + c);
        v[0] = t.x; v[1] = t.y; v[2] = t.z; v[3] = t.w;
      } else {
#pragma unroll
        for (int k = 0; k < 4; ++k)
          if (c + k < C) v[k] = x[r * C + c + k];
      }
      if (hi) {
        float h[4], l[4];
#pragma unroll
        for (int k = 0; k < 4; ++k) {
          h[k] = to_tf32(v[k]);
          l[k] = to_tf32(v[k] - h[k]);
        }
        if (c < ldp) {
          *reinterpret_cast<float4*>(hi + r * ldp + c) = make_float4(h[0], h[1], h[2], h[3]);
          *reinterpret_cast<float4*>(lo + r * ldp + c) = make_float4(l[0], l[1], l[2], l[3]);
        }
      }
    }
    if (hiT) {
#pragma unroll
      for (int k = 0; k < 4; ++k) tile[lr][tx * 4 + k] = v[k];
    }
  }
  if (!hiT) return;
  __syncthreads();
#pragma unroll
  for (int i = 0; i < 4; ++i) {
    const int lc = ty + 16 * i;
    const int64_t c = c0 + lc, r = r0 + tx * 4;
    if (c < C && r < ldt) {
      float h[4], l[4];
#pragma unroll
      for (int k = 0; k < 4; ++k) {
        const float v = tile[tx * 4 + k][lc];
        h[k] = to_tf32(v);
        l[k] = to_tf32(v - h[k]);
      }
      *reinterpret_cast<float4*>(hiT + c * ldt + r) = make_float4(h[0], h[1], h[2], h[3]);
      *reinterpret_cast<float4*>(loT + c * ldt + r) = make_float4(l[0], l[1], l[2], l[3]);
    }
  }
}

__device__ __forceinline__ void split_mix_body(const float* __restrict__ x, int64_t R, int64_t C,
                                               float* __restrict__ hi, __nv_bfloat16* __restrict__ h16,
                                               __nv_bfloat16* __restrict__ l16, int64_t ld, int vec_in,
                                               int relu_mode) {
  const int64_t gpr = ld / 8;
  const int64_t total = R * gpr;
  const int64_t stride = (int64_t)gridDim.x * blockDim.x;
  for (int64_t i = (int64_t)blockIdx.x * blockDim.x + threadIdx.x; i < total; i += stride) {
    const int64_t r = i / gpr, c = (i - r * gpr) * 8;
    float v[8];
    if (vec_in && c + 7 < C) {
      const float4 t0 = *reinterpret_cast<const float4*>(x + r * C + c);
      const float4 t1 = *reinterpret_cast<const float4*>(x + r * C + c + 4);
      v[0] = t0.x; v[1] = t0.y; v[2] = t0.z; v[3] = t0.w;
      v[4] = t1.x; v[5] = t1.y; v[6] = t1.z; v[7] = t1.w;
    } else {
#pragma unroll
      for (int k = 0; k < 8; ++k) v[k] = (c + k < C) ? x[r * C + c + k] : 0.f;
    }
    if (relu_mode) {
#pragma unroll
      for (int k = 0; k < 8; ++k) v[k] = v[k] < 0.f ? 0.f : v[k];
    }
    float h[8];
    union { __nv_bfloat162 b[4]; uint4 u; } ph, pl;
#pragma unroll
    for (int k = 0; k < 8; ++k) h[k] = to_tf32(v[k]);
#pragma unroll
    for (int k = 0; k < 4; ++k) {
      ph.b[k] = __floats2bfloat162_rn(v[2 * k], v[2 * k + 1]);
      pl.b[k] = __floats2bfloat162_rn(v[2 * k] - h[2 * k], v[2 * k + 1] - h[2 * k + 1]);
    }
    float* hp = hi + r * ld + c;
    *reinterpret_cast<float4*>(hp) = make_float4(h[0], h[1], h[2], h[3]);
    *reinterpret_cast<float4*>(hp + 4) = make_float4(h[4], h[5], h[6], h[7]);
    *reinterpret_cast<uint4*>(h16 + r * ld + c) = ph.u;
    *reinterpret_cast<uint4*>(l16 + r * ld + c) = pl.u;
  }
}

__global__ void __launch_bounds__(256)
split_mix_kernel(const float* __restrict__ x, int64_t R, int64_t C, float* __restrict__ hi,
                 __nv_bfloat16* __restrict__ h16, __nv_bfloat16* __restrict__ l16, int64_t ld,
                 int vec_in) {
  split_mix_body(x, R, C, hi, h16, l16, ld, vec_in, 0);
}

struct SplitArgs {
  const float* x; int64_t R, C; float* hi; __nv_bfloat16* h16; __nv_bfloat16* l16; int64_t ld;
  int vec_in, relu_mode;
};
__global__ void __launch_bounds__(256)
split_mix_cond2_kernel(SplitArgs a, SplitArgs b, const int* __restrict__ cond_a,
                       const int* __restrict__ cond_b, unsigned int* __restrict__ result_meta) {
  if (cond_a[3] && cond_b[3]) return;
  if (result_meta != nullptr && blockIdx.x == 0 && blockIdx.y == 0 && threadIdx.x == 0) result_meta[1] = 1u;
  const SplitArgs& s = blockIdx.y == 0 ? a : b;
  split_mix_body(s.x, s.R, s.C, s.hi, s.h16, s.l16, s.ld, s.vec_in, s.relu_mode);
}

static PFN_cuTensorMapEncodeTiled_v12000 g_encode = nullptr;

static int get_encode_fn() {
  if (g_encode) return 0;
  void* fn = nullptr;
  cudaDriverEntryPointQueryResult qres;
  TNN_CUDA(cudaGetDriverEntryPointByVersion("cuTensorMapEncodeTiled", &fn, 12000, cudaEnableDefault, &qres));
  if (qres != cudaDriverEntryPointSuccess || !fn) TNN_FAIL("cuTensorMapEncodeTiled is not available");
  g_encode = (PFN_cuTensorMapEncodeTiled_v12000)fn;
  return 0;
}

static int make_map(CUtensorMap* map, const float* ptr, int64_t rows, int64_t K, int64_t ld, int box_rows,
                    bool mn_major) {
  if ((reinterpret_cast<uintptr_t>(ptr) & 15) != 0) TNN_FAIL("tf32x3 GEMM: operand plane must be 16-byte aligned");
  if (ld % 4 != 0) TNN_FAIL("tf32x3 GEMM: operand pitch must be a multiple of 4 elements");
  cuuint64_t dims[2] = {(cuuint64_t)(mn_major ? rows : K), (cuuint64_t)(mn_major ? K : rows)};
  cuuint64_t strides[1] = {(cuuint64_t)ld * 4};
  cuuint32_t box[2] = {(cuuint32_t)(mn_major ? 32 : BK), (cuuint32_t)(mn_major ? BK : box_rows)};
  cuuint32_t estr[2] = {1, 1};
  CUresult r = g_encode(map, CU_TENSOR_MAP_DATA_TYPE_FLOAT32, 2, (void*)ptr, dims, strides, box, estr,
                        CU_TENSOR_MAP_INTERLEAVE_NONE,
                        mn_major ? CU_TENSOR_MAP_SWIZZLE_128B_ATOM_32B : CU_TENSOR_MAP_SWIZZLE_128B,
                        CU_TENSOR_MAP_L2_PROMOTION_L2_256B, CU_TENSOR_MAP_FLOAT_OOB_FILL_NONE);
  if (r != CUDA_SUCCESS) TNN_FAIL("cuTensorMapEncodeTiled failed with code " + std::to_string((int)r));
  return 0;
}

static int make_map16(CUtensorMap* map, const void* ptr, int64_t rows, int64_t K, int64_t ld, int box_rows,
                      bool mn_major) {
  if ((reinterpret_cast<uintptr_t>(ptr) & 15) != 0) TNN_FAIL("mixed GEMM: bf16 plane must be 16-byte aligned");
  if (ld % 8 != 0) TNN_FAIL("mixed GEMM: bf16 plane pitch must be a multiple of 8 elements");
  cuuint64_t dims[2] = {(cuuint64_t)(mn_major ? rows : K), (cuuint64_t)(mn_major ? K : rows)};
  cuuint64_t strides[1] = {(cuuint64_t)ld * 2};
  cuuint32_t box[2] = {(cuuint32_t)(mn_major ? 64 : BK), (cuuint32_t)(mn_major ? BK : box_rows)};
  cuuint32_t estr[2] = {1, 1};
  CUresult r = g_encode(map, CU_TENSOR_MAP_DATA_TYPE_BFLOAT16, 2, (void*)ptr, dims, strides, box, estr,
                        CU_TENSOR_MAP_INTERLEAVE_NONE,
                        mn_major ? CU_TENSOR_MAP_SWIZZLE_128B : CU_TENSOR_MAP_SWIZZLE_64B,
                        CU_TENSOR_MAP_L2_PROMOTION_L2_256B, CU_TENSOR_MAP_FLOAT_OOB_FILL_NONE);
  if (r != CUDA_SUCCESS) TNN_FAIL("cuTensorMapEncodeTiled (bf16) failed with code " + std::to_string((int)r));
  return 0;
}

constexpr int DEFAULT_CG = 2;
static unsigned int* g_tile_flags = nullptr;
constexpr int MAX_FLAG_TILES = 1 << 16;
static int g_group_m = 1;
static int g_force_ksplit = 0;
static int g_force_cg = 0;
static bool g_attr_set[3][2][2][2] = {};
int g_reserved_sms = 0;
static int g_exp_flags = 0;

struct ActOut {
  float* out = nullptr;
  float* hi = nullptr;
  float* lo = nullptr;
  void* l16 = nullptr;
  int64_t ld = 0;
  const float* mask_src = nullptr;
};

struct Planes {
  const float* hi;
  const void* lo;
  const void* l16;
  int64_t ld;
};

template <int CG, bool A_MN, bool B_MN, bool MIX>
static int launch_gemm(float* D, int64_t ldd, const Planes& a, const Planes& b, int64_t M, int64_t N,
                       int64_t K, const float* bias, int flags, const ActOut& act,
                       const int* cond_a = nullptr, const int* cond_b = nullptr) {
  using C = Cfg<CG>;
  CUtensorMap ma_hi, ma_lo, ma_l16, mb_hi, mb_lo, mb_l16;
  if (make_map(&ma_hi, a.hi, M, K, a.ld, ROWS_A, A_MN)) return 1;
  if (make_map(&mb_hi, b.hi, N, K, b.ld, C::ROWS_B, B_MN)) return 1;
  if constexpr (MIX) {
    if (make_map16(&ma_lo, a.lo, M, K, a.ld, ROWS_A, A_MN)) return 1;
    if (make_map16(&ma_l16, a.l16, M, K, a.ld, ROWS_A, A_MN)) return 1;
    if (make_map16(&mb_lo, b.lo, N, K, b.ld, C::ROWS_B, B_MN)) return 1;
    if (make_map16(&mb_l16, b.l16, N, K, b.ld, C::ROWS_B, B_MN)) return 1;
  } else {
    if (make_map(&ma_lo, (const float*)a.lo, M, K, a.ld, ROWS_A, A_MN)) return 1;
    if (make_map(&mb_lo, (const float*)b.lo, N, K, b.ld, C::ROWS_B, B_MN)) return 1;
    ma_l16 = ma_lo;
    mb_l16 = mb_lo;
  }
  auto kern = gemm_tf32x3_kernel<CG, A_MN, B_MN, MIX>;
  if (!g_attr_set[CG][A_MN][B_MN][MIX]) {
    TNN_CUDA(cudaFuncSetAttribute(kern, cudaFuncAttributeMaxDynamicSharedMemorySize, C::SMEM_BYTES));
    g_attr_set[CG][A_MN][B_MN][MIX] = true;
  }
  const int64_t tiles = ceil_div(M, C::TILE_M) * ceil_div(N, UMMA_N);
  const int usable_sms = std::max(CG, ctx().sm_count - g_reserved_sms);
  const int max_groups = usable_sms / CG;
  int t_full = (int)tiles, tail_split = 1;
  if (!(flags & 2) && tiles <= MAX_FLAG_TILES && g_force_ksplit != 1) {
    const int64_t num_kb = ceil_div(K, BK);
    if (g_force_ksplit > 1) {
      if (num_kb / g_force_ksplit >= 1) {
        t_full = 0;
        tail_split = g_force_ksplit;
      }
    } else {
      const int64_t rem = tiles % max_groups;
      if (rem > 0) {
        int s = 1;
        while (s < 4 && rem * (s * 2) <= max_groups && num_kb / (s * 2) >= 16) s *= 2;
        if (s > 1) {
          t_full = (int)(tiles - rem);
          tail_split = s;
        }
      }
    }
  }
  if (tail_split > 1) {
    if (!g_tile_flags) TNN_CUDA(cudaMalloc(&g_tile_flags, MAX_FLAG_TILES * sizeof(unsigned int)));
    TNN_CUDA(cudaMemsetAsync(g_tile_flags, 0, (size_t)tiles * sizeof(unsigned int), ctx().stream));
  }
  const int64_t units = t_full + (tiles - t_full) * tail_split;
  int groups = (int)std::min<int64_t>(units, max_groups);
  cudaLaunchConfig_t cfg = {};
  cfg.gridDim = dim3((unsigned)(groups * CG));
  cfg.blockDim = dim3(NUM_THREADS);
  cfg.dynamicSmemBytes = C::SMEM_BYTES;
  cfg.stream = ctx().stream;
  cudaLaunchAttribute attr[1];
  attr[0].id = cudaLaunchAttributeClusterDimension;
  attr[0].val.clusterDim.x = CG;
  attr[0].val.clusterDim.y = 1;
  attr[0].val.clusterDim.z = 1;
  cfg.attrs = attr;
  cfg.numAttrs = 1;
  const int family = cond_a ? 4 : 1;
  prof_begin(family);
  TNN_CUDA(cudaLaunchKernelEx(&cfg, kern, ma_hi, ma_lo, ma_l16, mb_hi, mb_lo, mb_l16, D, ldd, (int)M, (int)N, (int)K, bias, flags | g_exp_flags, t_full, tail_split, g_tile_flags, g_group_m,
                              act.out, act.hi, act.lo, (__nv_bfloat16*)act.l16, act.ld, act.mask_src, cond_a, cond_b));
  ctx().launches++;
  prof_end(family);
  return 0;
}

// ... 186 lines not shown
```

### tinynn-autograd_b200/csrc/reduce.cu

```cuda
#include <algorithm>
#include <cstdlib>
#include <type_traits>

#include "common.cuh"
#include "math.cuh"

namespace tnn {

template <int RED, typename T>
__device__ __forceinline__ T red_identity() {
  if constexpr (RED == TNN_RED_SUM) return T(0);
  else if constexpr (RED == TNN_RED_MAX) return -INFINITY;
  else return INFINITY;
}

template <int RED, typename T>
__device__ __forceinline__ T red_op(T a, T b) {
  if constexpr (RED == TNN_RED_SUM) return a + b;
  else if constexpr (RED == TNN_RED_MAX) return m_max(a, b);
  else return m_min(a, b);
}

template <int RED, typename T>
__device__ __forceinline__ T warp_reduce(T v) {
#pragma unroll
  for (int o = 16; o > 0; o >>= 1) v = red_op<RED, T>(v, __shfl_xor_sync(0xffffffffu, v, o));
  return v;
}

template <int RED, typename T>
__device__ __forceinline__ T block_reduce_256(T v) {
  __shared__ T sm[8];
  v = warp_reduce<RED, T>(v);
  const int lane = threadIdx.x & 31, w = threadIdx.x >> 5;
  if (lane == 0) sm[w] = v;
  __syncthreads();
  T r = red_identity<RED, T>();
  if (w == 0) {
    r = lane < 8 ? sm[lane] : red_identity<RED, T>();
#pragma unroll
    for (int o = 4; o > 0; o >>= 1) r = red_op<RED, T>(r, __shfl_xor_sync(0xffffffffu, r, o));
  }
  __syncthreads();
  return r;
}

template <int RED, typename T>
__global__ void __launch_bounds__(256)
reduce_row_block_kernel(T* out, const T* x, int64_t red, int nsplit) {
  const int64_t o = blockIdx.x;
  const int s = blockIdx.y;
  const int64_t chunk = ceil_div(red, nsplit);
  const int64_t lo = (int64_t)s * chunk;
  int64_t hi = lo + chunk;
  if (hi > red) hi = red;
  const T* row = x + o * red;
  T acc = red_identity<RED, T>();
  T a0 = acc, a1 = acc, a2 = acc, a3 = acc;
  int64_t i = lo + threadIdx.x;
  for (; i + 768 < hi; i += 1024) {
    T v0 = row[i], v1 = row[i + 256], v2 = row[i + 512], v3 = row[i + 768];
    a0 = red_op<RED, T>(a0, v0);
    a1 = red_op<RED, T>(a1, v1);
    a2 = red_op<RED, T>(a2, v2);
    a3 = red_op<RED, T>(a3, v3);
  }
  for (; i < hi; i += 256) a0 = red_op<RED, T>(a0, row[i]);
  acc = red_op<RED, T>(red_op<RED, T>(a0, a1), red_op<RED, T>(a2, a3));
  acc = block_reduce_256<RED, T>(acc);
  if (threadIdx.x == 0) out[o * nsplit + s] = acc;
}

template <int RED, typename T>
__global__ void __launch_bounds__(256)
reduce_row_warp_kernel(T* out, const T* x, int64_t outer, int64_t red) {
  const int lane = threadIdx.x & 31;
  const int64_t warps_total = (int64_t)gridDim.x * 8;
  for (int64_t o = (int64_t)blockIdx.x * 8 + (threadIdx.x >> 5); o < outer; o += warps_total) {
    const T* row = x + o * red;
    T acc = red_identity<RED, T>();
    for (int64_t i = lane; i < red; i += 32) acc = red_op<RED, T>(acc, row[i]);
    acc = warp_reduce<RED, T>(acc);
    if (lane == 0) out[o] = acc;
  }
}

template <int RED, typename T, int VEC>
__device__ __forceinline__ void col_accumulate(const T* __restrict__ base, int64_t lo, int64_t hi,
                                               int64_t inner, int ty, T (&acc)[VEC]) {
  using V = typename std::conditional<VEC == 1, T, typename std::conditional<sizeof(T) == 4, float4, double2>::type>::type;
  union U {
    V v;
    T e[VEC];
  };
  int64_t r = lo + ty;
  for (; r + 56 < hi; r += 64) {
    U u[8];
#pragma unroll
    for (int i = 0; i < 8; ++i) u[i].v = *reinterpret_cast<const V*>(base + (r + 8 * i) * inner);
#pragma unroll
    for (int i = 0; i < 8; ++i)
#pragma unroll
      for (int k = 0; k < VEC; ++k) acc[k] = red_op<RED, T>(acc[k], u[i].e[k]);
  }
  if (r < hi) {
    U u[8];
#pragma unroll
    for (int i = 0; i < 8; ++i)
      if (r + 8 * i < hi) u[i].v = *reinterpret_cast<const V*>(base + (r + 8 * i) * inner);
#pragma unroll
    for (int i = 0; i < 8; ++i)
      if (r + 8 * i < hi) {
#pragma unroll
        for (int k = 0; k < VEC; ++k) acc[k] = red_op<RED, T>(acc[k], u[i].e[k]);
      }
  }
}

template <int RED, typename T, int VEC>
__global__ void __launch_bounds__(256)
reduce_col_kernel(T* out, T* stage, const T* x, int64_t red, int64_t inner, int nsplit,
                  unsigned int* counters) {
  __shared__ T sm[8][32 * VEC + 1];
  __shared__ bool is_last;
  const int tx = threadIdx.x & 31, ty = threadIdx.x >> 5;
  const int64_t ncol = inner / VEC;
  const int64_t col = (int64_t)blockIdx.x * 32 + tx;
  const int64_t o = blockIdx.y / nsplit;
  const int s = blockIdx.y % nsplit;
  const int64_t chunk = ceil_div(red, nsplit);
  const int64_t lo = (int64_t)s * chunk;
  int64_t hi = lo + chunk;
  if (hi > red) hi = red;
  T acc[VEC];
#pragma unroll
  for (int k = 0; k < VEC; ++k) acc[k] = red_identity<RED, T>();
  if (col < ncol) col_accumulate<RED, T, VEC>(x + (o * red) * inner + col * VEC, lo, hi, inner, ty, acc);
#pragma unroll
  for (int k = 0; k < VEC; ++k) sm[ty][tx * VEC + k] = acc[k];
  __syncthreads();
  T* dst1 = nsplit > 1 ? stage + ((o * nsplit + s) * inner) : out + o * inner;
  if (ty == 0 && col < ncol) {
#pragma unroll
    for (int k = 0; k < VEC; ++k) {
      T r = sm[0][tx * VEC + k];
#pragma unroll
      for (int j = 1; j < 8; ++j) r = red_op<RED, T>(r, sm[j][tx * VEC + k]);
      dst1[col * VEC + k] = r;
    }
  }
  if (nsplit == 1) return;
  __threadfence();
  __syncthreads();
  if (threadIdx.x == 0) {
    unsigned int* cnt = counters + o * gridDim.x + blockIdx.x;
    const unsigned int prev = atomicAdd(cnt, 1u);
    is_last = prev == (unsigned int)nsplit - 1;
    if (is_last) *cnt = 0u;
  }
  __syncthreads();
  if (!is_last) return;
  __threadfence();
#pragma unroll
  for (int k = 0; k < VEC; ++k) acc[k] = red_identity<RED, T>();
  if (col < ncol)
    col_accumulate<RED, T, VEC>(stage + (o * nsplit) * inner + col * VEC, 0, nsplit, inner, ty, acc);
  __syncthreads();
#pragma unroll
  for (int k = 0; k < VEC; ++k) sm[ty][tx * VEC + k] = acc[k];
  __syncthreads();
  if (ty == 0 && col < ncol) {
#pragma unroll
    for (int k = 0; k < VEC; ++k) {
      T r = sm[0][tx * VEC + k];
#pragma unroll
      for (int j = 1; j < 8; ++j) r = red_op<RED, T>(r, sm[j][tx * VEC + k]);
      out[o * inner + col * VEC + k] = r;
    }
  }
}

static unsigned int* g_col_counters = nullptr;
constexpr int64_t MAX_COL_COUNTERS = 1 << 16;

template <int RED, typename T>
static int reduce_impl(T* out, const T* x, int64_t outer, int64_t red, int64_t inner) {
  Context& c = ctx();
  cudaStream_t st = c.stream;
  if (outer * inner == 0) return 0;
  if (red == 0) {
    if (RED != TNN_RED_SUM) TNN_FAIL("tnn_reduce: zero-size reduction has no identity");
    return tnn_fill(sizeof(T) == 4 ? TNN_F32 : TNN_F64, out, 0.0, outer * inner);
  }
  const int64_t target_ctas = (int64_t)c.sm_count * 4;
  if (inner == 1) {
    if (red <= 2048 && outer >= 64) {
      int grid = (int)std::min<int64_t>(ceil_div(outer, 8), (int64_t)c.sm_count * 8);
      reduce_row_warp_kernel<RED, T><<<grid, 256, 0, st>>>(out, x, outer, red);
      TNN_POST_LAUNCH();
      return 0;
    }
    int64_t nsplit = 1;
    if (outer < target_ctas) {
      nsplit = std::min<int64_t>(ceil_div(target_ctas, outer), ceil_div(red, 4096));
      if (nsplit < 1) nsplit = 1;
      if (nsplit > 65535) nsplit = 65535;
    }
    if (outer > 2147483647LL) TNN_FAIL("tnn_reduce: too many rows");
    if (nsplit == 1) {
      reduce_row_block_kernel<RED, T><<<dim3((unsigned)outer, 1), 256, 0, st>>>(out, x, red, 1);
      TNN_POST_LAUNCH();
      return 0;
    }
    void* scratch;
    if (get_scratch((size_t)(outer * nsplit) * sizeof(T), &scratch)) return 1;
    reduce_row_block_kernel<RED, T>
        <<<dim3((unsigned)outer, (unsigned)nsplit), 256, 0, st>>>((T*)scratch, x, red, (int)nsplit);
    TNN_POST_LAUNCH();
    if (outer >= 64) {
      int grid = (int)std::min<int64_t>(ceil_div(outer, 8), (int64_t)c.sm_count * 8);
      reduce_row_warp_kernel<RED, T><<<grid, 256, 0, st>>>(out, (const T*)scratch, outer, nsplit);
    } else {
      reduce_row_block_kernel<RED, T>
          <<<dim3((unsigned)outer, 1), 256, 0, st>>>(out, (const T*)scratch, nsplit, 1);
    }
    TNN_POST_LAUNCH();
    return 0;
  }
  constexpr int VW = sizeof(T) == 4 ? 4 : 2;
  bool vec = (inner % VW == 0) && ((reinterpret_cast<uintptr_t>(x) & 15) == 0);
  int64_t ncol = vec ? inner / VW : inner;
  int64_t gx = ceil_div(ncol, 32);
  int64_t nsplit = 1;
  if (gx * outer < target_ctas && outer * red * inner > (int64_t(1) << 18)) {
    static int col_ctas_per_sm = -1;
    if (col_ctas_per_sm < 0) {
      const char* e = getenv("TNN_COLSUM_CTAS_PER_SM");
      col_ctas_per_sm = e ? atoi(e) : 3;
      if (col_ctas_per_sm < 1) col_ctas_per_sm = 1;
    }
    const int64_t want = (int64_t)c.sm_count * col_ctas_per_sm;
    nsplit = std::min<int64_t>(ceil_div(want, gx * outer), ceil_div(red, 64));
    if (nsplit < 1) nsplit = 1;
  }
  if (outer * nsplit > 65535) {
    nsplit = std::max<int64_t>(1, 65535 / outer);
    if (outer > 65535) TNN_FAIL("tnn_reduce: outer extent above 65535 with inner > 1 is not supported");
  }
  void* scratch = nullptr;
  if (nsplit > 1) {
    if (gx * outer > MAX_COL_COUNTERS) nsplit = 1;
    else if (get_scratch((size_t)(outer * nsplit * inner) * sizeof(T), &scratch)) return 1;
  }
  if (nsplit > 1 && !g_col_counters) {
    TNN_CUDA(cudaMalloc(&g_col_counters, MAX_COL_COUNTERS * sizeof(unsigned int)));
    TNN_CUDA(cudaMemsetAsync(g_col_counters, 0, MAX_COL_COUNTERS * sizeof(unsigned int), st));
  }
  dim3 grid((unsigned)gx, (unsigned)(outer * nsplit));
  if (vec)
    reduce_col_kernel<RED, T, VW><<<grid, 256, 0, st>>>(out, (T*)scratch, x, red, inner, (int)nsplit, g_col_counters);
  else
    reduce_col_kernel<RED, T, 1><<<grid, 256, 0, st>>>(out, (T*)scratch, x, red, inner, (int)nsplit, g_col_counters);
  TNN_POST_LAUNCH();
  return 0;
}

template <typename T>
static int reduce_dispatch(int red_op_code, T* out, const T* x, int64_t outer, int64_t red,
                           int64_t inner) {
  switch (red_op_code) {
    case TNN_RED_SUM:
      return reduce_impl<TNN_RED_SUM, T>(out, x, outer, red, inner);
    case TNN_RED_MAX:
      return reduce_impl<TNN_RED_MAX, T>(out, x, outer, red, inner);
    case TNN_RED_MIN:
      return reduce_impl<TNN_RED_MIN, T>(out, x, outer, red, inner);
  }
  TNN_FAIL("tnn_reduce: unknown reduction code");
}

}

using namespace tnn;

extern "C" {

int tnn_reduce(int red_op_code, int dtype, void* out, const void* x, int64_t outer, int64_t red,
               int64_t inner) {
  TNN_REQUIRE_INIT();
  if (outer < 0 || red < 0 || inner < 0) TNN_FAIL("tnn_reduce: negative extent");
  if (dtype == TNN_F32)
    return reduce_dispatch<float>(red_op_code, (float*)out, (const float*)x, outer, red, inner);
  if (dtype == TNN_F64)
    return reduce_dispatch<double>(red_op_code, (double*)out, (const double*)x, outer, red, inner);
  TNN_FAIL("tnn_reduce: dtype must be TNN_F32 or TNN_F64");
}

int tnn_colsum(int dtype, void* out, const void* g, int64_t R, int64_t C) {
  return tnn_reduce(TNN_RED_SUM, dtype, out, g, 1, R, C);
}

int tnn_unbroadcast(int dtype, void* out, const void* grad, int ndim, const int64_t* gshape,
                    const int32_t* keep) {
  TNN_REQUIRE_INIT();
  if (ndim < 0 || ndim > TNN_MAX_DIMS) TNN_FAIL("tnn_unbroadcast: rank above TNN_MAX_DIMS");
  const size_t esz = dtype == TNN_F32 ? 4 : 8;
  if (dtype != TNN_F32 && dtype != TNN_F64) TNN_FAIL("tnn_unbroadcast: bad dtype");
  int64_t dims[TNN_MAX_DIMS];
  int kp[TNN_MAX_DIMS];
  int n = 0;
  for (int d = 0; d < ndim; ++d) {
    if (gshape[d] == 1) continue;
    int k = keep[d] ? 1 : 0;
    if (n > 0 && kp[n - 1] == k) dims[n - 1] *= gshape[d];
    else {
      dims[n] = gshape[d];
      kp[n] = k;
      ++n;
    }
  }
  int64_t total = 1;
  for (int i = 0; i < n; ++i) total *= dims[i];
  const void* cur = grad;
  void* tmp_prev = nullptr;
  while (true) {
    int g = -1;
    for (int i = 0; i < n; ++i)
      if (!kp[i]) {
        g = i;
        break;
      }
    if (g < 0) {
      int rc = 0;
      if (cur != out) rc = tnn_d2d(out, cur, (size_t)total * esz);
      if (tmp_prev) tnn_free(tmp_prev);
      return rc;
    }
    int64_t outer = 1, inner = 1;
    for (int i = 0; i < g; ++i) outer *= dims[i];
    for (int i = g + 1; i < n; ++i) inner *= dims[i];
    bool last = true;
    for (int i = g + 1; i < n; ++i)
      if (!kp[i]) last = false;
    void* dst = out;
    void* tmp = nullptr;
    if (!last) {
      if (tnn_alloc((size_t)(outer * inner) * esz, &tmp)) return 1;
      dst = tmp;
    }
    int rc = tnn_reduce(TNN_RED_SUM, dtype, dst, cur, outer, dims[g], inner);
    if (tmp_prev) tnn_free(tmp_prev);
    if (rc) {
      if (tmp) tnn_free(tmp);
      return rc;
    }
    if (last) return 0;
    tmp_prev = tmp;
    cur = tmp;
    total /= dims[g];
    for (int i = g; i + 1 < n; ++i) {
      dims[i] = dims[i + 1];
      kp[i] = kp[i + 1];
    }
    --n;
    if (g > 0 && g < n && kp[g - 1] == kp[g]) {
      dims[g - 1] *= dims[g];
      for (int i = g; i + 1 < n; ++i) {
        dims[i] = dims[i + 1];
        kp[i] = kp[i + 1];
      }
      --n;
    }
  }
}

}
```

### tinynn-autograd_b200/csrc/tc_ptx.cuh

```cuda
#pragma once
#include <cuda.h>
#include <cuda_bf16.h>
#include <cstdint>
#include <cstdio>

namespace tnn {
namespace tc {

__device__ __forceinline__ uint32_t smem_u32(const void* p) {
  return (uint32_t)__cvta_generic_to_shared(p);
}
__device__ __forceinline__ void mbar_init(uint32_t bar, uint32_t count) {
  asm volatile("mbarrier.init.shared::cta.b64 [%0], %1;" ::"r"(bar), "r"(count) : "memory");
}
__device__ __forceinline__ void mbar_expect_tx(uint32_t bar, uint32_t bytes) {
  asm volatile("mbarrier.arrive.expect_tx.shared::cta.b64 _, [%0], %1;" ::"r"(bar), "r"(bytes)
               : "memory");
}
__device__ __forceinline__ void mbar_arrive(uint32_t bar) {
  asm volatile("mbarrier.arrive.shared::cta.b64 _, [%0];" ::"r"(bar) : "memory");
}
__device__ __forceinline__ void mbar_arrive_cluster(uint32_t bar, uint32_t cta) {
  asm volatile(
      "{\n\t.reg .b32 ra;\n\t"
// ... 7 lines not shown
#pragma unroll 1
  for (uint32_t spin = 0;; ++spin) {
    asm volatile(
        "{\n\t.reg .pred p;\n\t"
        "mbarrier.try_wait.parity.shared::cta.b64 p, [%1], %2;\n\t"
        "selp.u32 %0, 1, 0, p;\n\t}"
        : "=r"(done) : "r"(bar), "r"(parity) : "memory");
    if (done) return;
    if (spin == 0) t0 = clock64();
    else if (clock64() - t0 > 4000000000LL) break;
  }
  printf("tnn gemm_tc: mbarrier wait timed out (block %d thread %d bar %x parity %u)\n",
         (int)blockIdx.x, (int)threadIdx.x, bar, parity);
  __trap();
}
__device__ __forceinline__ void mbar_arrive_cluster_relaxed(uint32_t bar, uint32_t cta) {
  asm volatile(
      "{\n\t.reg .b32 ra;\n\t"
      "mapa.shared::cluster.u32 ra, %0, %1;\n\t"
      "mbarrier.arrive.relaxed.cluster.shared::cluster.b64 _, [ra];\n\t}"
      ::"r"(bar), "r"(cta) : "memory");
}
__device__ __forceinline__ void fence_barrier_init() {
  asm volatile("fence.mbarrier_init.release.cluster;" ::: "memory");
}
__device__ __forceinline__ void fence_proxy_async() {
  asm volatile("fence.proxy.async.shared::cta;" ::: "memory");
}
__device__ __forceinline__ void cluster_sync_all() {
  asm volatile("barrier.cluster.arrive.release.aligned;\n\tbarrier.cluster.wait.acquire.aligned;"
               ::: "memory");
}
__device__ __forceinline__ uint32_t cluster_ctarank() {
  uint32_t r;
  asm volatile("mov.u32 %0, %%cluster_ctarank;" : "=r"(r));
  return r;
}
__device__ __forceinline__ void tma_prefetch_desc(const CUtensorMap* m) {
  asm volatile("prefetch.tensormap [%0];" ::"l"(m) : "memory");
}
template <int CG>
__device__ __forceinline__ void tma_load_2d(uint32_t dst, const CUtensorMap* map, uint32_t bar,
                                            int c0, int c1) {
  if constexpr (CG == 1) {
    asm volatile(
        "cp.async.bulk.tensor.2d.shared::cluster.global.tile.mbarrier::complete_tx::bytes"
        " [%0], [%1, {%3, %4}], [%2];"
        ::"r"(dst), "l"(map), "r"(bar), "r"(c0), "r"(c1) : "memory");
  } else {
    asm volatile(
        "cp.async.bulk.tensor.2d.cta_group::2.shared::cluster.global.tile.mbarrier::complete_tx::bytes"
        " [%0], [%1, {%3, %4}], [%2];"
        ::"r"(dst), "l"(map), "r"(bar & 0xFEFFFFFFu), "r"(c0), "r"(c1) : "memory");
  }
}
__device__ __forceinline__ void tma_load_2d_pair_mc(uint32_t dst, const CUtensorMap* map, uint32_t bar,
                                                    int c0, int c1, uint16_t mask) {
  asm volatile(
      "cp.async.bulk.tensor.2d.cta_group::2.shared::cluster.global.tile.mbarrier::complete_tx::bytes"
      ".multicast::cluster [%0], [%1, {%4, %5}], [%2], %3;"
      ::"r"(dst), "l"(map), "r"(bar & 0xFEFFFFFFu), "h"(mask), "r"(c0), "r"(c1) : "memory");
}
__device__ __forceinline__ void umma_commit_pair_mask(uint32_t bar, uint16_t mask) {
  asm volatile(
      "tcgen05.commit.cta_group::2.mbarrier::arrive::one.shared::cluster.multicast::cluster.b64 [%0], %1;"
      ::"r"(bar), "h"(mask) : "memory");
}
__device__ __forceinline__ void tma_prefetch_l2_2d(const CUtensorMap* map, int c0, int c1) {
  asm volatile("cp.async.bulk.prefetch.tensor.2d.L2.global.tile [%0, {%1, %2}];"
               ::"l"(map), "r"(c0), "r"(c1) : "memory");
}
template <int CG>
__device__ __forceinline__ void tmem_alloc(uint32_t dst_smem, uint32_t cols) {
  if constexpr (CG == 1)
    asm volatile("tcgen05.alloc.cta_group::1.sync.aligned.shared::cta.b32 [%0], %1;" ::"r"(dst_smem), "r"(cols) : "memory");
  else
    asm volatile("tcgen05.alloc.cta_group::2.sync.aligned.shared::cta.b32 [%0], %1;" ::"r"(dst_smem), "r"(cols) : "memory");
}
template <int CG>
__device__ __forceinline__ void tmem_relinquish() {
  if constexpr (CG == 1) asm volatile("tcgen05.relinquish_alloc_permit.cta_group::1.sync.aligned;" ::: "memory");
  else asm volatile("tcgen05.relinquish_alloc_permit.cta_group::2.sync.aligned;" ::: "memory");
}
template <int CG>
__device__ __forceinline__ void tmem_dealloc(uint32_t taddr, uint32_t cols) {
  if constexpr (CG == 1) asm volatile("tcgen05.dealloc.cta_group::1.sync.aligned.b32 %0, %1;" ::"r"(taddr), "r"(cols) : "memory");
  else asm volatile("tcgen05.dealloc.cta_group::2.sync.aligned.b32 %0, %1;" ::"r"(taddr), "r"(cols) : "memory");
}
__device__ __forceinline__ void tc_fence_before() {
  asm volatile("tcgen05.fence::before_thread_sync;" ::: "memory");
}
__device__ __forceinline__ void tc_fence_after() {
  asm volatile("tcgen05.fence::after_thread_sync;" ::: "memory");
}
template <int CG>
__device__ __forceinline__ void umma_tf32(uint32_t tmem_d, uint64_t adesc, uint64_t bdesc,
                                          uint32_t idesc, uint32_t accumulate) {
  if constexpr (CG == 1)
    asm volatile(
        "{\n\t.reg .pred p;\n\tsetp.ne.b32 p, %4, 0;\n\t"
        "tcgen05.mma.cta_group::1.kind::tf32 [%0], %1, %2, %3, p;\n\t}"
        ::"r"(tmem_d), "l"(adesc), "l"(bdesc), "r"(idesc), "r"(accumulate) : "memory");
  else
    asm volatile(
        "{\n\t.reg .pred p;\n\tsetp.ne.b32 p, %4, 0;\n\t"
        "tcgen05.mma.cta_group::2.kind::tf32 [%0], %1, %2, %3, p;\n\t}"
        ::"r"(tmem_d), "l"(adesc), "l"(bdesc), "r"(idesc), "r"(accumulate) : "memory");
}
template <int CG>
__device__ __forceinline__ void umma_bf16(uint32_t tmem_d, uint64_t adesc, uint64_t bdesc,
                                          uint32_t idesc, uint32_t accumulate) {
  if constexpr (CG == 1)
    asm volatile(
        "{\n\t.reg .pred p;\n\tsetp.ne.b32 p, %4, 0;\n\t"
        "tcgen05.mma.cta_group::1.kind::f16 [%0], %1, %2, %3, p;\n\t}"
        ::"r"(tmem_d), "l"(adesc), "l"(bdesc), "r"(idesc), "r"(accumulate) : "memory");
  else
    asm volatile(
        "{\n\t.reg .pred p;\n\tsetp.ne.b32 p, %4, 0;\n\t"
        "tcgen05.mma.cta_group::2.kind::f16 [%0], %1, %2, %3, p;\n\t}"
        ::"r"(tmem_d), "l"(adesc), "l"(bdesc), "r"(idesc), "r"(accumulate) : "memory");
}
template <int CG>
__device__ __forceinline__ void umma_commit(uint32_t bar) {
  if constexpr (CG == 1)
    asm volatile("tcgen05.commit.cta_group::1.mbarrier::arrive::one.shared::cluster.b64 [%0];" ::"r"(bar) : "memory");
  else
    asm volatile(
        "tcgen05.commit.cta_group::2.mbarrier::arrive::one.shared::cluster.multicast::cluster.b64 [%0], %1;"
        ::"r"(bar), "h"((uint16_t)3) : "memory");
}
__device__ __forceinline__ void tmem_ld_32x32b_x32(uint32_t taddr, uint32_t (&r)[32]) {
  asm volatile(
      "tcgen05.ld.sync.aligned.32x32b.x32.b32 "
      "{%0, %1, %2, %3, %4, %5, %6, %7, %8, %9, %10, %11, %12, %13, %14, %15, "
      "%16, %17, %18, %19, %20, %21, %22, %23, %24, %25, %26, %27, %28, %29, %30, %31}, [%32];"
      : "=r"(r[0]), "=r"(r[1]), "=r"(r[2]), "=r"(r[3]), "=r"(r[4]), "=r"(r[5]), "=r"(r[6]),
        "=r"(r[7]), "=r"(r[8]), "=r"(r[9]), "=r"(r[10]), "=r"(r[11]), "=r"(r[12]), "=r"(r[13]),
        "=r"(r[14]), "=r"(r[15]), "=r"(r[16]), "=r"(r[17]), "=r"(r[18]), "=r"(r[19]), "=r"(r[20]),
        "=r"(r[21]), "=r"(r[22]), "=r"(r[23]), "=r"(r[24]), "=r"(r[25]), "=r"(r[26]), "=r"(r[27]),
        "=r"(r[28]), "=r"(r[29]), "=r"(r[30]), "=r"(r[31])
      : "r"(taddr) : "memory");
}
__device__ __forceinline__ void tmem_ld_wait() {
  asm volatile("tcgen05.wait::ld.sync.aligned;" ::: "memory");
}

__device__ __forceinline__ float to_tf32(float x) {
  uint32_t r;
  asm("cvt.rna.tf32.f32 %0, %1;" : "=r"(r) : "f"(x));
  return __uint_as_float(r);
}

}
}
```

Measured before the change: 1.051 million.

## Fuse fp16 split with bias-grad colsum and fold fallback split into GEMM

Adds a split_f16_colsum kernel that produces the fp16 hi/lo planes and the column sum in one read of the gradient, caching the colsum so the later bias-gradient reduction is skipped. It also moves the fallback tf32/bf16 split into the f16x3 GEMM kernel, which runs it only when the scale check fails, removing a separate launch per GEMM. The colsum reduction helpers are factored into a shared header. This adds complexity to the early-exit path of the GEMM kernel and depends on the split cache being invalidated correctly, for example in add_inplace.

Result: faster. 1.071 million (median of 6 runs) (+1.9%).

```diff
diff --git a/core/_backend.py b/core/_backend.py
--- a/core/_backend.py
+++ b/core/_backend.py
@@ -99,8 +99,13 @@
     "tnn_set_gemm_f16_cluster": [_c_int],
     "tnn_f16_meta_reset": [_c_vp],
     "tnn_split_f16": [_c_vp, _c_i64, _c_i64, _c_vp, _c_vp, _c_i64, _c_vp, _c_int],
+    "tnn_split_f16_colsum": [_c_vp, _c_i64, _c_i64, _c_vp, _c_vp, _c_i64, _c_vp, _c_vp],
     "tnn_gemm_f16x3": [_c_vp, _c_i64, _c_vp, _c_vp, _c_i64, _c_vp, _c_vp, _c_vp, _c_i64, _c_vp, _c_i64,
                        _c_i64, _c_i64, _c_vp, _c_int, _c_int, _c_vp, _c_vp, _c_vp],
+    "tnn_gemm_f16x3_fb": [_c_vp, _c_i64, _c_vp, _c_vp, _c_i64, _c_vp, _c_vp, _c_vp, _c_i64, _c_vp, _c_i64,
+                          _c_i64, _c_i64, _c_vp, _c_int, _c_int, _c_vp, _c_vp, _c_vp,
+                          _c_vp, _c_i64, _c_i64, _c_vp, _c_vp, _c_vp, _c_int,
+                          _c_vp, _c_i64, _c_i64, _c_vp, _c_vp, _c_vp, _c_int],
     "tnn_split_tf32_bf16_cond": [_c_vp, _c_i64, _c_i64, _c_vp, _c_vp, _c_vp, _c_i64, _c_int,
                                  _c_vp, _c_i64, _c_i64, _c_vp, _c_vp, _c_vp, _c_i64, _c_int, _c_vp, _c_vp, _c_vp],
     "tnn_f16_stats_cond": [_c_vp, _c_i64, _c_vp, _c_int],
@@ -591,6 +596,7 @@
 
 
 def add_inplace(dst, src):
+    dst.split = None
     if src.dtype != dst.dtype:
         src = astype(src, dst.dtype)
     if _lib.tnn_ew_flat(ADD, _DT_CODE[dst.dtype], dst.ptr, dst.ptr, src.ptr, None, dst.size,
@@ -659,6 +665,12 @@
 
 def colsum(g, out=None):
     R, C = g.shape
+    cache = g.split
+    if cache is not None and cache.get("epoch") == _split_epoch and "colsum" in cache:
+        if out is None:
+            return clone(cache["colsum"])
+        copy_into(out, cache["colsum"])
+        return out
     if out is None:
         out = empty((1, C), g.dtype)
     if _lib.tnn_colsum(_DT_CODE[g.dtype], out.ptr, g.ptr, R, C):
@@ -804,7 +816,12 @@
     elif _lib.tnn_f16_stats_cond(src.ptr, R * C, meta.ptr, relu_mode):
         _raise("tnn_f16_stats_cond")
     hf, l16 = _empty_16bit(R, ld), _empty_16bit(R, ld)
-    if _lib.tnn_split_f16(src.ptr, R, C, hf.ptr, l16.ptr, ld, meta.ptr, relu_mode):
+    if cache.get("want_colsum") and relu_mode == 0:
+        cs = empty((1, C), F32)
+        if _lib.tnn_split_f16_colsum(src.ptr, R, C, hf.ptr, l16.ptr, ld, meta.ptr, cs.ptr):
+            _raise("tnn_split_f16_colsum")
+        cache["colsum"] = cs
+    elif _lib.tnn_split_f16(src.ptr, R, C, hf.ptr, l16.ptr, ld, meta.ptr, relu_mode):
         _raise("tnn_split_f16")
     cache["f"] = (hf, l16, ld, meta, src if src is not x else None, relu_mode)
     return cache["f"]
@@ -852,18 +869,15 @@
     real_act = act_out if (act and type(act_out) is not LazyReLU) else None
     bias_p = bias.ptr if bias is not None else None
     mask_p = mask_src.ptr if (act and mask_src is not None) else None
-    if _lib.tnn_gemm_f16x3(out.ptr, N, a_hf.ptr, a_l16.ptr, lda, a_meta.ptr, b_hf.ptr, b_l16.ptr, ldb,
-                           b_meta.ptr, M, N, K, bias_p, flags, layout,
-                           real_act.ptr if real_act is not None else None, mask_p,
-                           stat.ptr if stat is not None else None):
-        _raise("tnn_gemm_f16x3")
     fa = _fallback_planes(0, a.shape[0], lda)
     fb = _fallback_planes(1, b.shape[0], ldb)
-    if _lib.tnn_split_tf32_bf16_cond(a_src.ptr, a.shape[0], a.shape[1], fa[0].ptr, fa[1].ptr, fa[2].ptr, lda,
-                                     a_relu, b_src.ptr, b.shape[0], b.shape[1], fb[0].ptr, fb[1].ptr,
-                                     fb[2].ptr, ldb, b_relu, a_meta.ptr, b_meta.ptr,
-                                     stat.ptr if stat is not None else None):
-        _raise("tnn_split_tf32_bf16_cond")
+    if _lib.tnn_gemm_f16x3_fb(out.ptr, N, a_hf.ptr, a_l16.ptr, lda, a_meta.ptr, b_hf.ptr, b_l16.ptr, ldb,
+                              b_meta.ptr, M, N, K, bias_p, flags, layout,
+                              real_act.ptr if real_act is not None else None, mask_p,
+                              stat.ptr if stat is not None else None,
+                              a_src.ptr, a.shape[0], a.shape[1], fa[0].ptr, fa[1].ptr, fa[2].ptr, a_relu,
+                              b_src.ptr, b.shape[0], b.shape[1], fb[0].ptr, fb[1].ptr, fb[2].ptr, b_relu):
+        _raise("tnn_gemm_f16x3_fb")
     if _lib.tnn_gemm_tf32_bf16x2_cond(out.ptr, N, fa[0].ptr, fa[1].ptr, fa[2].ptr, lda, fb[0].ptr, fb[1].ptr,
                                       fb[2].ptr, ldb, M, N, K, bias_p, flags & 3, layout,
                                       real_act.ptr if real_act is not None else None, mask_p,
@@ -871,6 +885,8 @@
         _raise("tnn_gemm_tf32_bf16x2_cond")
     if act:
         act_out.split = {"epoch": _split_epoch, "stat": stat}
+        if mask_src is not None:
+            act_out.split["want_colsum"] = True
         return out, act_out
     return out
 
@@ -1119,7 +1135,7 @@
                        q.ptr, float(m_global), g.ptr, stat.ptr if stat is not None else None, lab_ptr):
         _raise("tnn_ce_bwd")
     if stat is not None:
-        dz.split = {"epoch": _split_epoch, "stat": stat}
+        dz.split = {"epoch": _split_epoch, "stat": stat, "want_colsum": True}
     return dz
 
 
diff --git a/include/tnn_b200.h b/include/tnn_b200.h
--- a/include/tnn_b200.h
+++ b/include/tnn_b200.h
@@ -148,10 +148,18 @@
 int tnn_f16_meta_reset(void* meta);
 int tnn_split_f16(const float* x, int64_t R, int64_t C, void* hf, void* l16, int64_t ld, void* meta,
                   int relu_mode);
+int tnn_split_f16_colsum(const float* x, int64_t R, int64_t C, void* hf, void* l16, int64_t ld, void* meta,
+                         float* colsum_out);
 int tnn_gemm_f16x3(float* D, int64_t ldd, const void* a_hf, const void* a_l16, int64_t lda,
                    const void* a_meta, const void* b_hf, const void* b_l16, int64_t ldb,
                    const void* b_meta, int64_t M, int64_t N, int64_t K, const float* bias, int flags,
                    int layout, float* act_out, const float* mask_src, void* stat_meta);
+int tnn_gemm_f16x3_fb(float* D, int64_t ldd, const void* a_hf, const void* a_l16, int64_t lda,
+                      const void* a_meta, const void* b_hf, const void* b_l16, int64_t ldb,
+                      const void* b_meta, int64_t M, int64_t N, int64_t K, const float* bias, int flags,
+                      int layout, float* act_out, const float* mask_src, void* stat_meta,
+                      const float* xa, int64_t Ra, int64_t Ca, float* hia, void* h16a, void* l16a, int relu_a,
+                      const float* xb, int64_t Rb, int64_t Cb, float* hib, void* h16b, void* l16b, int relu_b);
 int tnn_split_tf32_bf16_cond(const float* xa, int64_t Ra, int64_t Ca, float* hia, void* h16a, void* l16a,
                              int64_t lda, int relu_a, const float* xb, int64_t Rb, int64_t Cb, float* hib,
                              void* h16b, void* l16b, int64_t ldb, int relu_b, const void* meta_a,
diff --git a/tinynn-autograd_b200/build.py b/tinynn-autograd_b200/build.py
--- a/tinynn-autograd_b200/build.py
+++ b/tinynn-autograd_b200/build.py
@@ -12,7 +12,8 @@
 
 SOURCES = ["runtime.cu", "elementwise.cu", "reduce.cu", "layout.cu", "gemm_simt.cu",
            "gemm_tc.cu", "gemm_f16.cu", "fused.cu", "mlp_fused.cu", "comm.cu"]
-HEADERS = [os.path.join(CSRC, "common.cuh"), os.path.join(CSRC, "math.cuh"), os.path.join(CSRC, "tc_ptx.cuh"),
+HEADERS = [os.path.join(CSRC, "common.cuh"), os.path.join(CSRC, "math.cuh"), os.path.join(CSRC, "reduce.cuh"),
+           os.path.join(CSRC, "tc_ptx.cuh"),
            os.path.join(ROOT, "include", "tnn_b200.h")]
 
 NVCC_FLAGS = ["-gencode", "arch=compute_100a,code=sm_100a", "-O3", "-lineinfo", "-std=c++17",
diff --git a/tinynn-autograd_b200/csrc/gemm_f16.cu b/tinynn-autograd_b200/csrc/gemm_f16.cu
--- a/tinynn-autograd_b200/csrc/gemm_f16.cu
+++ b/tinynn-autograd_b200/csrc/gemm_f16.cu
@@ -7,6 +7,7 @@
 #include <cstdlib>
 
 #include "common.cuh"
+#include "reduce.cuh"
 #include "tc_ptx.cuh"
 
 namespace tnn {
@@ -142,8 +143,16 @@
                   const float* __restrict__ bias, int flags, int t_full, int tail_split,
                   unsigned int* __restrict__ tile_flags, float* __restrict__ act_out,
                   const float* __restrict__ mask_src, const Meta* __restrict__ meta_a,
-                  const Meta* __restrict__ meta_b, Meta* __restrict__ stat_out, int group_m) {
-  if (!(meta_a->safe && meta_b->safe)) return;
+                  const Meta* __restrict__ meta_b, Meta* __restrict__ stat_out, int group_m,
+                  const SplitArgs fb_a, const SplitArgs fb_b) {
+  if (!(meta_a->safe && meta_b->safe)) {
+    if (fb_a.x != nullptr) {
+      if (stat_out != nullptr && blockIdx.x == 0 && threadIdx.x == 0) stat_out->need_stats = 1u;
+      split_mix_body(fb_a.x, fb_a.R, fb_a.C, fb_a.hi, fb_a.h16, fb_a.l16, fb_a.ld, fb_a.vec_in, fb_a.relu_mode);
+      split_mix_body(fb_b.x, fb_b.R, fb_b.C, fb_b.hi, fb_b.h16, fb_b.l16, fb_b.ld, fb_b.vec_in, fb_b.relu_mode);
+    }
+    return;
+  }
   extern __shared__ uint8_t smem_raw[];
   const uint32_t smem_base = (smem_u32(smem_raw) + 1023u) & ~1023u;
   uint8_t* smem_gen = smem_raw + (smem_base - smem_u32(smem_raw));
@@ -643,6 +652,44 @@
   }
 }
 
+__device__ __forceinline__ void split_counts(float a, unsigned int& n_small, unsigned int& n_nz) {
+  n_nz += (a != 0.f);
+  n_small += (a != 0.f && fabsf(a) < SMALL_LIMIT);
+}
+
+__device__ __forceinline__ void split_pair(float a, float b, __half2& h, __half2& l, unsigned int& n_small,
+                                           unsigned int& n_nz) {
+  split_counts(a, n_small, n_nz);
+  split_counts(b, n_small, n_nz);
+  h = __floats2half2_rn(a, b);
+  const float2 hb = __half22float2(h);
+  l = __floats2half2_rn(a - hb.x, b - hb.y);
+}
+
+__device__ __forceinline__ void split_finish(Meta* meta, unsigned int n_small, unsigned int n_nz, int e, int ok,
+                                             unsigned int n_ctas) {
+  n_small = __reduce_add_sync(0xFFFFFFFFu, n_small);
+  n_nz = __reduce_add_sync(0xFFFFFFFFu, n_nz);
+  __shared__ unsigned int s_small[8], s_nz[8];
+  const int warp = threadIdx.x >> 5, lane = threadIdx.x & 31;
+  if (lane == 0) { s_small[warp] = n_small; s_nz[warp] = n_nz; }
+  __syncthreads();
+  if (threadIdx.x == 0) {
+#pragma unroll
+    for (int w = 1; w < 8; ++w) { n_small += s_small[w]; n_nz += s_nz[w]; }
+    if (n_small) atomicAdd(&meta->n_small, n_small);
+    if (n_nz) atomicAdd(&meta->n_nz, n_nz);
+    __threadfence();
+    if (atomicAdd(&meta->ticket, 1u) == n_ctas - 1) {
+      __threadfence();
+      const unsigned int ts = *reinterpret_cast<volatile unsigned int*>(&meta->n_small);
+      const unsigned int tn = *reinterpret_cast<volatile unsigned int*>(&meta->n_nz);
+      meta->exp = e;
+      meta->safe = (ok && (unsigned long long)ts * GUARD_FRACTION <= (unsigned long long)tn) ? 1 : 0;
+    }
+  }
+}
+
 __global__ void __launch_bounds__(256)
 split_f16_kernel(const float* __restrict__ x, int64_t R, int64_t C, __half* __restrict__ hf,
                  __half* __restrict__ l16, int64_t ld, Meta* __restrict__ meta, int relu_mode,
@@ -672,37 +719,91 @@
       for (int k = 0; k < 4; ++k) {
         float a = v[2 * k], b = v[2 * k + 1];
         if (relu_mode) { a = a < 0.f ? 0.f : a; b = b < 0.f ? 0.f : b; }
-        a *= sc; b *= sc;
-        n_nz += (a != 0.f) + (b != 0.f);
-        n_small += (a != 0.f && fabsf(a) < SMALL_LIMIT) + (b != 0.f && fabsf(b) < SMALL_LIMIT);
-        const __half2 h = __floats2half2_rn(a, b);
-        const float2 hb = __half22float2(h);
-        ph.h[k] = h;
-        pl.h[k] = __floats2half2_rn(a - hb.x, b - hb.y);
+        split_pair(a * sc, b * sc, ph.h[k], pl.h[k], n_small, n_nz);
       }
       *reinterpret_cast<uint4*>(hf + r * ld + c) = ph.u;
       *reinterpret_cast<uint4*>(l16 + r * ld + c) = pl.u;
     }
   }
-  n_small = __reduce_add_sync(0xFFFFFFFFu, n_small);
-  n_nz = __reduce_add_sync(0xFFFFFFFFu, n_nz);
-  __shared__ unsigned int s_small[8], s_nz[8];
-  const int warp = threadIdx.x >> 5, lane = threadIdx.x & 31;
-  if (lane == 0) { s_small[warp] = n_small; s_nz[warp] = n_nz; }
+  split_finish(meta, n_small, n_nz, e, ok, gridDim.x);
+}
+
+template <int VEC>
+__global__ void __launch_bounds__(256)
+split_f16_colsum_kernel(const float* __restrict__ x, int64_t R, int64_t C, __half* __restrict__ hf,
+                        __half* __restrict__ l16, int64_t ld, Meta* __restrict__ meta, float* __restrict__ out,
+                        float* __restrict__ stage, int nsplit, unsigned int* __restrict__ counters) {
+  __shared__ float sm[8][32 * VEC + 1];
+  __shared__ bool is_last;
+  int e, ok;
+  meta_scale(meta->absmax, e, ok);
+  const float sc = ok ? pow2f(e) : 1.f;
+  const int tx = threadIdx.x & 31, ty = threadIdx.x >> 5;
+  const int64_t ncol = C / VEC;
+  const int64_t col = (int64_t)blockIdx.x * 32 + tx;
+  const int s = blockIdx.y;
+  const int64_t chunk = ceil_div(R, nsplit);
+  const int64_t lo = (int64_t)s * chunk;
+  int64_t hi = lo + chunk;
+  if (hi > R) hi = R;
+  unsigned int n_small = 0u, n_nz = 0u;
+  float acc[VEC];
+#pragma unroll
+  for (int k = 0; k < VEC; ++k) acc[k] = 0.f;
+  if (col < ncol) {
+    const int64_t c0 = col * VEC;
+    const bool last_slot = col == ncol - 1;
+    auto visit = [&](int64_t r, const float (&v)[VEC]) {
+      if (!ok) return;
+      if constexpr (VEC == 4) {
+        union { __half2 h[2]; uint2 u; } ph, pl;
+        split_pair(v[0] * sc, v[1] * sc, ph.h[0], pl.h[0], n_small, n_nz);
+        split_pair(v[2] * sc, v[3] * sc, ph.h[1], pl.h[1], n_small, n_nz);
+        *reinterpret_cast<uint2*>(hf + r * ld + c0) = ph.u;
+        *reinterpret_cast<uint2*>(l16 + r * ld + c0) = pl.u;
+      } else {
+        const float a = v[0] * sc;
+        split_counts(a, n_small, n_nz);
+        const __half h = __float2half_rn(a);
+        hf[r * ld + c0] = h;
+        l16[r * ld + c0] = __float2half_rn(a - __half2float(h));
+      }
+      if (last_slot)
+        for (int64_t c = C; c < ld; ++c) {
+          hf[r * ld + c] = __float2half_rn(0.f);
+          l16[r * ld + c] = __float2half_rn(0.f);
+        }
+    };
+    col_accumulate<TNN_RED_SUM, float, VEC>(x + c0, lo, hi, C, ty, acc, visit);
+  }
+  split_finish(meta, n_small, n_nz, e, ok, gridDim.x * gridDim.y);
+  __syncthreads();
+  col_fold_lanes<TNN_RED_SUM, float, VEC>(sm, tx, ty, acc);
+  float* dst1 = nsplit > 1 ? stage + (int64_t)s * C : out;
+  if (ty == 0 && col < ncol) {
+#pragma unroll
+    for (int k = 0; k < VEC; ++k) dst1[col * VEC + k] = acc[k];
+  }
+  if (nsplit == 1) return;
+  __threadfence();
   __syncthreads();
   if (threadIdx.x == 0) {
-#pragma unroll
-    for (int w = 1; w < 8; ++w) { n_small += s_small[w]; n_nz += s_nz[w]; }
-    if (n_small) atomicAdd(&meta->n_small, n_small);
-    if (n_nz) atomicAdd(&meta->n_nz, n_nz);
-    __threadfence();
-    if (atomicAdd(&meta->ticket, 1u) == gridDim.x - 1) {
-      __threadfence();
-      const unsigned int ts = *reinterpret_cast<volatile unsigned int*>(&meta->n_small);
-      const unsigned int tn = *reinterpret_cast<volatile unsigned int*>(&meta->n_nz);
-      meta->exp = e;
-      meta->safe = (ok && (unsigned long long)ts * GUARD_FRACTION <= (unsigned long long)tn) ? 1 : 0;
-    }
+    unsigned int* cnt = counters + blockIdx.x;
+    const unsigned int prev = atomicAdd(cnt, 1u);
+    is_last = prev == (unsigned int)nsplit - 1;
+    if (is_last) *cnt = 0u;
+  }
+  __syncthreads();
+  if (!is_last) return;
+  __threadfence();
+#pragma unroll
+  for (int k = 0; k < VEC; ++k) acc[k] = 0.f;
+  if (col < ncol) col_accumulate<TNN_RED_SUM, float, VEC>(stage + col * VEC, 0, nsplit, C, ty, acc);
+  __syncthreads();
+  col_fold_lanes<TNN_RED_SUM, float, VEC>(sm, tx, ty, acc);
+  if (ty == 0 && col < ncol) {
+#pragma unroll
+    for (int k = 0; k < VEC; ++k) out[col * VEC + k] = acc[k];
   }
 }
 
@@ -746,7 +847,7 @@
 static int launch(float* D, int64_t ldd, const void* a_h, const void* a_l, int64_t lda, const void* b_h,
                   const void* b_l, int64_t ldb, int64_t M, int64_t N, int64_t K, const float* bias,
                   int flags, float* act_out, const float* mask_src, const Meta* meta_a,
-                  const Meta* meta_b, Meta* stat_out) {
+                  const Meta* meta_b, Meta* stat_out, const SplitArgs& fb_a, const SplitArgs& fb_b) {
   CUtensorMap ma_h, ma_l, mb_h, mb_l;
   if (make_map(&ma_h, a_h, M, K, lda, A_MN, CL == 4 ? 64 : KBOX_ROWS)) return 1;
   if (make_map(&ma_l, a_l, M, K, lda, A_MN, CL == 4 ? 64 : KBOX_ROWS)) return 1;
@@ -802,7 +903,8 @@
   const int gm = (CL == 4 && g_group_m < 0) ? std::min(-1, g_group_m / 2) : g_group_m;
   prof_begin(1);
   TNN_CUDA(cudaLaunchKernelEx(&cfg, kern, ma_h, ma_l, mb_h, mb_l, D, ldd, (int)M, (int)N, (int)K, bias, flags,
-                              t_full, tail_split, g_tile_flags, act_out, mask_src, meta_a, meta_b, stat_out, gm));
+                              t_full, tail_split, g_tile_flags, act_out, mask_src, meta_a, meta_b, stat_out, gm,
+                              fb_a, fb_b));
   ctx().launches++;
   prof_end(1);
   return 0;
@@ -812,12 +914,12 @@
 static int launch_layout(int layout, float* D, int64_t ldd, const void* a_h, const void* a_l, int64_t lda,
                          const void* b_h, const void* b_l, int64_t ldb, int64_t M, int64_t N, int64_t K,
                          const float* bias, int flags, float* act_out, const float* mask_src,
-                         const Meta* ma, const Meta* mb, Meta* st) {
+                         const Meta* ma, const Meta* mb, Meta* st, const SplitArgs& fa, const SplitArgs& fb) {
   switch (layout & 3) {
-    case 0: return launch<false, false, CL>(D, ldd, a_h, a_l, lda, b_h, b_l, ldb, M, N, K, bias, flags, act_out, mask_src, ma, mb, st);
-    case 1: return launch<true, false, CL>(D, ldd, a_h, a_l, lda, b_h, b_l, ldb, M, N, K, bias, flags, act_out, mask_src, ma, mb, st);
-    case 2: return launch<false, true, CL>(D, ldd, a_h, a_l, lda, b_h, b_l, ldb, M, N, K, bias, flags, act_out, mask_src, ma, mb, st);
-    default: return launch<true, true, CL>(D, ldd, a_h, a_l, lda, b_h, b_l, ldb, M, N, K, bias, flags, act_out, mask_src, ma, mb, st);
+    case 0: return launch<false, false, CL>(D, ldd, a_h, a_l, lda, b_h, b_l, ldb, M, N, K, bias, flags, act_out, mask_src, ma, mb, st, fa, fb);
+    case 1: return launch<true, false, CL>(D, ldd, a_h, a_l, lda, b_h, b_l, ldb, M, N, K, bias, flags, act_out, mask_src, ma, mb, st, fa, fb);
+    case 2: return launch<false, true, CL>(D, ldd, a_h, a_l, lda, b_h, b_l, ldb, M, N, K, bias, flags, act_out, mask_src, ma, mb, st, fa, fb);
+    default: return launch<true, true, CL>(D, ldd, a_h, a_l, lda, b_h, b_l, ldb, M, N, K, bias, flags, act_out, mask_src, ma, mb, st, fa, fb);
   }
 }
 
@@ -881,10 +983,35 @@
   return 0;
 }
 
-int tnn_gemm_f16x3(float* D, int64_t ldd, const void* a_hf, const void* a_l16, int64_t lda,
-                   const void* a_meta, const void* b_hf, const void* b_l16, int64_t ldb,
-                   const void* b_meta, int64_t M, int64_t N, int64_t K, const float* bias, int flags,
-                   int layout, float* act_out, const float* mask_src, void* stat_meta) {
+int tnn_split_f16_colsum(const float* x, int64_t R, int64_t C, void* hf, void* l16, int64_t ld, void* meta,
+                         float* colsum_out) {
+  TNN_REQUIRE_INIT();
+  if (R <= 0 || C <= 0) return 0;
+  if (!hf || !l16 || !meta || !colsum_out) TNN_FAIL("tnn_split_f16_colsum: both planes, the meta record and the sum vector are required");
+  if (ld % 8 != 0 || ld < C) TNN_FAIL("tnn_split_f16_colsum: ld must be >= C and a multiple of 8");
+  const bool vec = (C % 4 == 0) && ((reinterpret_cast<uintptr_t>(x) & 15) == 0);
+  ColPlan plan;
+  if (col_plan(1, R, C, sizeof(float), vec, plan)) return 1;
+  const dim3 grid((unsigned)plan.gx, (unsigned)plan.nsplit);
+  prof_begin(3);
+  if (vec)
+    f16::split_f16_colsum_kernel<4><<<grid, 256, 0, ctx().stream>>>(
+        x, R, C, (__half*)hf, (__half*)l16, ld, (f16::Meta*)meta, colsum_out, (float*)plan.scratch,
+        (int)plan.nsplit, plan.counters);
+  else
+    f16::split_f16_colsum_kernel<1><<<grid, 256, 0, ctx().stream>>>(
+        x, R, C, (__half*)hf, (__half*)l16, ld, (f16::Meta*)meta, colsum_out, (float*)plan.scratch,
+        (int)plan.nsplit, plan.counters);
+  TNN_POST_LAUNCH();
+  prof_end(3);
+  return 0;
+}
+
+static int gemm_f16x3_impl(float* D, int64_t ldd, const void* a_hf, const void* a_l16, int64_t lda,
+                           const void* a_meta, const void* b_hf, const void* b_l16, int64_t ldb,
+                           const void* b_meta, int64_t M, int64_t N, int64_t K, const float* bias, int flags,
+                           int layout, float* act_out, const float* mask_src, void* stat_meta,
+                           const tc::SplitArgs& fa, const tc::SplitArgs& fb) {
   TNN_REQUIRE_INIT();
   if (M <= 0 || N <= 0) return 0;
   if (K <= 0) TNN_FAIL("tnn_gemm_f16x3: K must be positive");
@@ -909,8 +1036,35 @@
   const f16::Meta* mb = (const f16::Meta*)b_meta;
   f16::Meta* st = (f16::Meta*)stat_meta;
   if (f16::g_cluster == 4 && N > f16::UMMA_N)
-    return f16::launch_layout<4>(layout, D, ldd, a_hf, a_l16, lda, b_hf, b_l16, ldb, M, N, K, bias, flags, act_out, mask_src, ma, mb, st);
-  return f16::launch_layout<2>(layout, D, ldd, a_hf, a_l16, lda, b_hf, b_l16, ldb, M, N, K, bias, flags, act_out, mask_src, ma, mb, st);
-}
-
-}
+    return f16::launch_layout<4>(layout, D, ldd, a_hf, a_l16, lda, b_hf, b_l16, ldb, M, N, K, bias, flags, act_out, mask_src, ma, mb, st, fa, fb);
+  return f16::launch_layout<2>(layout, D, ldd, a_hf, a_l16, lda, b_hf, b_l16, ldb, M, N, K, bias, flags, act_out, mask_src, ma, mb, st, fa, fb);
+}
+
+int tnn_gemm_f16x3(float* D, int64_t ldd, const void* a_hf, const void* a_l16, int64_t lda,
+                   const void* a_meta, const void* b_hf, const void* b_l16, int64_t ldb,
+                   const void* b_meta, int64_t M, int64_t N, int64_t K, const float* bias, int flags,
+                   int layout, float* act_out, const float* mask_src, void* stat_meta) {
+  const tc::SplitArgs none = {};
+  return gemm_f16x3_impl(D, ldd, a_hf, a_l16, lda, a_meta, b_hf, b_l16, ldb, b_meta, M, N, K, bias, flags,
+                         layout, act_out, mask_src, stat_meta, none, none);
+}
+
+int tnn_gemm_f16x3_fb(float* D, int64_t ldd, const void* a_hf, const void* a_l16, int64_t lda,
+                      const void* a_meta, const void* b_hf, const void* b_l16, int64_t ldb,
+                      const void* b_meta, int64_t M, int64_t N, int64_t K, const float* bias, int flags,
+                      int layout, float* act_out, const float* mask_src, void* stat_meta,
+                      const float* xa, int64_t Ra, int64_t Ca, float* hia, void* h16a, void* l16a, int relu_a,
+                      const float* xb, int64_t Rb, int64_t Cb, float* hib, void* h16b, void* l16b, int relu_b) {
+  if (!xa || !xb || !hia || !h16a || !l16a || !hib || !h16b || !l16b)
+    TNN_FAIL("tnn_gemm_f16x3_fb: both fallback sources and all their planes are required");
+  if (Ra <= 0 || Ca <= 0 || Rb <= 0 || Cb <= 0 || lda < Ca || ldb < Cb)
+    TNN_FAIL("tnn_gemm_f16x3_fb: fallback operand extents do not fit the plane pitches");
+  const tc::SplitArgs fa{xa, Ra, Ca, hia, (__nv_bfloat16*)h16a, (__nv_bfloat16*)l16a, lda,
+                         (Ca % 4 == 0) && ((reinterpret_cast<uintptr_t>(xa) & 15) == 0), relu_a};
+  const tc::SplitArgs fb{xb, Rb, Cb, hib, (__nv_bfloat16*)h16b, (__nv_bfloat16*)l16b, ldb,
+                         (Cb % 4 == 0) && ((reinterpret_cast<uintptr_t>(xb) & 15) == 0), relu_b};
+  return gemm_f16x3_impl(D, ldd, a_hf, a_l16, lda, a_meta, b_hf, b_l16, ldb, b_meta, M, N, K, bias, flags,
+                         layout, act_out, mask_src, stat_meta, fa, fb);
+}
+
+}
diff --git a/tinynn-autograd_b200/csrc/gemm_tc.cu b/tinynn-autograd_b200/csrc/gemm_tc.cu
--- a/tinynn-autograd_b200/csrc/gemm_tc.cu
+++ b/tinynn-autograd_b200/csrc/gemm_tc.cu
@@ -667,46 +667,6 @@
   }
 }
 
-__device__ __forceinline__ void split_mix_body(const float* __restrict__ x, int64_t R, int64_t C,
-                                               float* __restrict__ hi, __nv_bfloat16* __restrict__ h16,
-                                               __nv_bfloat16* __restrict__ l16, int64_t ld, int vec_in,
-                                               int relu_mode) {
-  const int64_t gpr = ld / 8;
-  const int64_t total = R * gpr;
-  const int64_t stride = (int64_t)gridDim.x * blockDim.x;
-  for (int64_t i = (int64_t)blockIdx.x * blockDim.x + threadIdx.x; i < total; i += stride) {
-    const int64_t r = i / gpr, c = (i - r * gpr) * 8;
-    float v[8];
-    if (vec_in && c + 7 < C) {
-      const float4 t0 = *reinterpret_cast<const float4*>(x + r * C + c);
-      const float4 t1 = *reinterpret_cast<const float4*>(x + r * C + c + 4);
-      v[0] = t0.x; v[1] = t0.y; v[2] = t0.z; v[3] = t0.w;
-      v[4] = t1.x; v[5] = t1.y; v[6] = t1.z; v[7] = t1.w;
-    } else {
-#pragma unroll
-      for (int k = 0; k < 8; ++k) v[k] = (c + k < C) ? x[r * C + c + k] : 0.f;
-    }
-    if (relu_mode) {
-#pragma unroll
-      for (int k = 0; k < 8; ++k) v[k] = v[k] < 0.f ? 0.f : v[k];
-    }
-    float h[8];
-    union { __nv_bfloat162 b[4]; uint4 u; } ph, pl;
-#pragma unroll
-    for (int k = 0; k < 8; ++k) h[k] = to_tf32(v[k]);
-#pragma unroll
-    for (int k = 0; k < 4; ++k) {
-      ph.b[k] = __floats2bfloat162_rn(v[2 * k], v[2 * k + 1]);
-      pl.b[k] = __floats2bfloat162_rn(v[2 * k] - h[2 * k], v[2 * k + 1] - h[2 * k + 1]);
-    }
-    float* hp = hi + r * ld + c;
-    *reinterpret_cast<float4*>(hp) = make_float4(h[0], h[1], h[2], h[3]);
-    *reinterpret_cast<float4*>(hp + 4) = make_float4(h[4], h[5], h[6], h[7]);
-    *reinterpret_cast<uint4*>(h16 + r * ld + c) = ph.u;
-    *reinterpret_cast<uint4*>(l16 + r * ld + c) = pl.u;
-  }
-}
-
 __global__ void __launch_bounds__(256)
 split_mix_kernel(const float* __restrict__ x, int64_t R, int64_t C, float* __restrict__ hi,
                  __nv_bfloat16* __restrict__ h16, __nv_bfloat16* __restrict__ l16, int64_t ld,
@@ -714,10 +674,6 @@
   split_mix_body(x, R, C, hi, h16, l16, ld, vec_in, 0);
 }
 
-struct SplitArgs {
-  const float* x; int64_t R, C; float* hi; __nv_bfloat16* h16; __nv_bfloat16* l16; int64_t ld;
-  int vec_in, relu_mode;
-};
 __global__ void __launch_bounds__(256)
 split_mix_cond2_kernel(SplitArgs a, SplitArgs b, const int* __restrict__ cond_a,
                        const int* __restrict__ cond_b, unsigned int* __restrict__ result_meta) {
diff --git a/tinynn-autograd_b200/csrc/reduce.cu b/tinynn-autograd_b200/csrc/reduce.cu
--- a/tinynn-autograd_b200/csrc/reduce.cu
+++ b/tinynn-autograd_b200/csrc/reduce.cu
@@ -4,22 +4,9 @@
 
 #include "common.cuh"
 #include "math.cuh"
+#include "reduce.cuh"
 
 namespace tnn {
-
-template <int RED, typename T>
-__device__ __forceinline__ T red_identity() {
-  if constexpr (RED == TNN_RED_SUM) return T(0);
-  else if constexpr (RED == TNN_RED_MAX) return -INFINITY;
-  else return INFINITY;
-}
-
-template <int RED, typename T>
-__device__ __forceinline__ T red_op(T a, T b) {
-  if constexpr (RED == TNN_RED_SUM) return a + b;
-  else if constexpr (RED == TNN_RED_MAX) return m_max(a, b);
-  else return m_min(a, b);
-}
 
 template <int RED, typename T>
 __device__ __forceinline__ T warp_reduce(T v) {
@@ -86,38 +73,6 @@
 }
 
 template <int RED, typename T, int VEC>
-__device__ __forceinline__ void col_accumulate(const T* __restrict__ base, int64_t lo, int64_t hi,
-                                               int64_t inner, int ty, T (&acc)[VEC]) {
-  using V = typename std::conditional<VEC == 1, T, typename std::conditional<sizeof(T) == 4, float4, double2>::type>::type;
-  union U {
-    V v;
-    T e[VEC];
-  };
-  int64_t r = lo + ty;
-  for (; r + 56 < hi; r += 64) {
-    U u[8];
-#pragma unroll
-    for (int i = 0; i < 8; ++i) u[i].v = *reinterpret_cast<const V*>(base + (r + 8 * i) * inner);
-#pragma unroll
-    for (int i = 0; i < 8; ++i)
-#pragma unroll
-      for (int k = 0; k < VEC; ++k) acc[k] = red_op<RED, T>(acc[k], u[i].e[k]);
-  }
-  if (r < hi) {
-    U u[8];
-#pragma unroll
-    for (int i = 0; i < 8; ++i)
-      if (r + 8 * i < hi) u[i].v = *reinterpret_cast<const V*>(base + (r + 8 * i) * inner);
-#pragma unroll
-    for (int i = 0; i < 8; ++i)
-      if (r + 8 * i < hi) {
-#pragma unroll
-        for (int k = 0; k < VEC; ++k) acc[k] = red_op<RED, T>(acc[k], u[i].e[k]);
-      }
-  }
-}
-
-template <int RED, typename T, int VEC>
 __global__ void __launch_bounds__(256)
 reduce_col_kernel(T* out, T* stage, const T* x, int64_t red, int64_t inner, int nsplit,
                   unsigned int* counters) {
@@ -136,18 +91,11 @@
 #pragma unroll
   for (int k = 0; k < VEC; ++k) acc[k] = red_identity<RED, T>();
   if (col < ncol) col_accumulate<RED, T, VEC>(x + (o * red) * inner + col * VEC, lo, hi, inner, ty, acc);
-#pragma unroll
-  for (int k = 0; k < VEC; ++k) sm[ty][tx * VEC + k] = acc[k];
-  __syncthreads();
+  col_fold_lanes<RED, T, VEC>(sm, tx, ty, acc);
   T* dst1 = nsplit > 1 ? stage + ((o * nsplit + s) * inner) : out + o * inner;
   if (ty == 0 && col < ncol) {
 #pragma unroll
-    for (int k = 0; k < VEC; ++k) {
-      T r = sm[0][tx * VEC + k];
-#pragma unroll
-      for (int j = 1; j < 8; ++j) r = red_op<RED, T>(r, sm[j][tx * VEC + k]);
-      dst1[col * VEC + k] = r;
-    }
+    for (int k = 0; k < VEC; ++k) dst1[col * VEC + k] = acc[k];
   }
   if (nsplit == 1) return;
   __threadfence();
@@ -166,22 +114,52 @@
   if (col < ncol)
     col_accumulate<RED, T, VEC>(stage + (o * nsplit) * inner + col * VEC, 0, nsplit, inner, ty, acc);
   __syncthreads();
-#pragma unroll
-  for (int k = 0; k < VEC; ++k) sm[ty][tx * VEC + k] = acc[k];
-  __syncthreads();
+  col_fold_lanes<RED, T, VEC>(sm, tx, ty, acc);
   if (ty == 0 && col < ncol) {
 #pragma unroll
-    for (int k = 0; k < VEC; ++k) {
-      T r = sm[0][tx * VEC + k];
-#pragma unroll
-      for (int j = 1; j < 8; ++j) r = red_op<RED, T>(r, sm[j][tx * VEC + k]);
-      out[o * inner + col * VEC + k] = r;
-    }
+    for (int k = 0; k < VEC; ++k) out[o * inner + col * VEC + k] = acc[k];
   }
 }
 
 static unsigned int* g_col_counters = nullptr;
 constexpr int64_t MAX_COL_COUNTERS = 1 << 16;
+
+int col_plan(int64_t outer, int64_t red, int64_t inner, size_t elem_bytes, bool vec, ColPlan& plan) {
+  Context& c = ctx();
+  const int64_t target_ctas = (int64_t)c.sm_count * 4;
+  const int64_t ncol = vec ? inner / (int64_t)(16 / elem_bytes) : inner;
+  const int64_t gx = ceil_div(ncol, 32);
+  int64_t nsplit = 1;
+  if (gx * outer < target_ctas && outer * red * inner > (int64_t(1) << 18)) {
+    static int col_ctas_per_sm = -1;
+    if (col_ctas_per_sm < 0) {
+      const char* e = getenv("TNN_COLSUM_CTAS_PER_SM");
+      col_ctas_per_sm = e ? atoi(e) : 3;
+      if (col_ctas_per_sm < 1) col_ctas_per_sm = 1;
+    }
+    const int64_t want = (int64_t)c.sm_count * col_ctas_per_sm;
+    nsplit = std::min<int64_t>(ceil_div(want, gx * outer), ceil_div(red, 64));
+    if (nsplit < 1) nsplit = 1;
+  }
+  if (outer * nsplit > 65535) {
+    nsplit = std::max<int64_t>(1, 65535 / outer);
+    if (outer > 65535) TNN_FAIL("tnn_reduce: outer extent above 65535 with inner > 1 is not supported");
+  }
+  void* scratch = nullptr;
+  if (nsplit > 1) {
+    if (gx * outer > MAX_COL_COUNTERS) nsplit = 1;
+    else if (get_scratch((size_t)(outer * nsplit * inner) * elem_bytes, &scratch)) return 1;
+  }
+  if (nsplit > 1 && !g_col_counters) {
+    TNN_CUDA(cudaMalloc(&g_col_counters, MAX_COL_COUNTERS * sizeof(unsigned int)));
+    TNN_CUDA(cudaMemsetAsync(g_col_counters, 0, MAX_COL_COUNTERS * sizeof(unsigned int), c.stream));
+  }
+  plan.gx = gx;
+  plan.nsplit = nsplit;
+  plan.scratch = scratch;
+  plan.counters = g_col_counters;
+  return 0;
+}
 
 template <int RED, typename T>
 static int reduce_impl(T* out, const T* x, int64_t outer, int64_t red, int64_t inner) {
@@ -228,39 +206,16 @@
     return 0;
   }
   constexpr int VW = sizeof(T) == 4 ? 4 : 2;
-  bool vec = (inner % VW == 0) && ((reinterpret_cast<uintptr_t>(x) & 15) == 0);
-  int64_t ncol = vec ? inner / VW : inner;
-  int64_t gx = ceil_div(ncol, 32);
-  int64_t nsplit = 1;
-  if (gx * outer < target_ctas && outer * red * inner > (int64_t(1) << 18)) {
-    static int col_ctas_per_sm = -1;
-    if (col_ctas_per_sm < 0) {
-      const char* e = getenv("TNN_COLSUM_CTAS_PER_SM");
-      col_ctas_per_sm = e ? atoi(e) : 3;
-      if (col_ctas_per_sm < 1) col_ctas_per_sm = 1;
-    }
-    const int64_t want = (int64_t)c.sm_count * col_ctas_per_sm;
-    nsplit = std::min<int64_t>(ceil_div(want, gx * outer), ceil_div(red, 64));
-    if (nsplit < 1) nsplit = 1;
-  }
-  if (outer * nsplit > 65535) {
-    nsplit = std::max<int64_t>(1, 65535 / outer);
-    if (outer > 65535) TNN_FAIL("tnn_reduce: outer extent above 65535 with inner > 1 is not supported");
-  }
-  void* scratch = nullptr;
-  if (nsplit > 1) {
-    if (gx * outer > MAX_COL_COUNTERS) nsplit = 1;
-    else if (get_scratch((size_t)(outer * nsplit * inner) * sizeof(T), &scratch)) return 1;
-  }
-  if (nsplit > 1 && !g_col_counters) {
-    TNN_CUDA(cudaMalloc(&g_col_counters, MAX_COL_COUNTERS * sizeof(unsigned int)));
-    TNN_CUDA(cudaMemsetAsync(g_col_counters, 0, MAX_COL_COUNTERS * sizeof(unsigned int), st));
-  }
+  const bool vec = (inner % VW == 0) && ((reinterpret_cast<uintptr_t>(x) & 15) == 0);
+  ColPlan plan;
+  if (col_plan(outer, red, inner, sizeof(T), vec, plan)) return 1;
+  const int64_t gx = plan.gx, nsplit = plan.nsplit;
+  void* scratch = plan.scratch;
   dim3 grid((unsigned)gx, (unsigned)(outer * nsplit));
   if (vec)
-    reduce_col_kernel<RED, T, VW><<<grid, 256, 0, st>>>(out, (T*)scratch, x, red, inner, (int)nsplit, g_col_counters);
+    reduce_col_kernel<RED, T, VW><<<grid, 256, 0, st>>>(out, (T*)scratch, x, red, inner, (int)nsplit, plan.counters);
   else
-    reduce_col_kernel<RED, T, 1><<<grid, 256, 0, st>>>(out, (T*)scratch, x, red, inner, (int)nsplit, g_col_counters);
+    reduce_col_kernel<RED, T, 1><<<grid, 256, 0, st>>>(out, (T*)scratch, x, red, inner, (int)nsplit, plan.counters);
   TNN_POST_LAUNCH();
   return 0;
 }
diff --git a/tinynn-autograd_b200/csrc/reduce.cuh b/tinynn-autograd_b200/csrc/reduce.cuh
--- /dev/null
+++ b/tinynn-autograd_b200/csrc/reduce.cuh
@@ -0,0 +1,88 @@
+#pragma once
+#include <type_traits>
+
+#include "common.cuh"
+#include "math.cuh"
+
+namespace tnn {
+
+template <int RED, typename T>
+__device__ __forceinline__ T red_identity() {
+  if constexpr (RED == TNN_RED_SUM) return T(0);
+  else if constexpr (RED == TNN_RED_MAX) return -INFINITY;
+  else return INFINITY;
+}
+
+template <int RED, typename T>
+__device__ __forceinline__ T red_op(T a, T b) {
+  if constexpr (RED == TNN_RED_SUM) return a + b;
+  else if constexpr (RED == TNN_RED_MAX) return m_max(a, b);
+  else return m_min(a, b);
+}
+
+struct NoVisit {
+  template <typename T, int VEC>
+  __device__ __forceinline__ void operator()(int64_t, const T (&)[VEC]) const {}
+};
+
+template <int RED, typename T, int VEC, typename Visit = NoVisit>
+__device__ __forceinline__ void col_accumulate(const T* __restrict__ base, int64_t lo, int64_t hi,
+                                               int64_t inner, int ty, T (&acc)[VEC],
+                                               Visit visit = Visit()) {
+  using V = typename std::conditional<VEC == 1, T, typename std::conditional<sizeof(T) == 4, float4, double2>::type>::type;
+  union U {
+    V v;
+    T e[VEC];
+  };
+  int64_t r = lo + ty;
+  for (; r + 56 < hi; r += 64) {
+    U u[8];
+#pragma unroll
+    for (int i = 0; i < 8; ++i) u[i].v = *reinterpret_cast<const V*>(base + (r + 8 * i) * inner);
+#pragma unroll
+    for (int i = 0; i < 8; ++i) {
+      visit(r + 8 * i, u[i].e);
+#pragma unroll
+      for (int k = 0; k < VEC; ++k) acc[k] = red_op<RED, T>(acc[k], u[i].e[k]);
+    }
+  }
+  if (r < hi) {
+    U u[8];
+#pragma unroll
+    for (int i = 0; i < 8; ++i)
+      if (r + 8 * i < hi) u[i].v = *reinterpret_cast<const V*>(base + (r + 8 * i) * inner);
+#pragma unroll
+    for (int i = 0; i < 8; ++i)
+      if (r + 8 * i < hi) {
+        visit(r + 8 * i, u[i].e);
+#pragma unroll
+        for (int k = 0; k < VEC; ++k) acc[k] = red_op<RED, T>(acc[k], u[i].e[k]);
+      }
+  }
+}
+
+template <int RED, typename T, int VEC>
+__device__ __forceinline__ void col_fold_lanes(T (*sm)[32 * VEC + 1], int tx, int ty, T (&acc)[VEC]) {
+#pragma unroll
+  for (int k = 0; k < VEC; ++k) sm[ty][tx * VEC + k] = acc[k];
+  __syncthreads();
+  if (ty == 0) {
+#pragma unroll
+    for (int k = 0; k < VEC; ++k) {
+      T r = sm[0][tx * VEC + k];
+#pragma unroll
+      for (int j = 1; j < 8; ++j) r = red_op<RED, T>(r, sm[j][tx * VEC + k]);
+      acc[k] = r;
+    }
+  }
+}
+
+struct ColPlan {
+  int64_t gx = 0;
+  int64_t nsplit = 1;
+  void* scratch = nullptr;
+  unsigned int* counters = nullptr;
+};
+int col_plan(int64_t outer, int64_t red, int64_t inner, size_t elem_bytes, bool vec, ColPlan& plan);
+
+}
diff --git a/tinynn-autograd_b200/csrc/tc_ptx.cuh b/tinynn-autograd_b200/csrc/tc_ptx.cuh
--- a/tinynn-autograd_b200/csrc/tc_ptx.cuh
+++ b/tinynn-autograd_b200/csrc/tc_ptx.cuh
@@ -183,5 +183,50 @@
   return __uint_as_float(r);
 }
 
-}
-}
+__device__ __forceinline__ void split_mix_body(const float* __restrict__ x, int64_t R, int64_t C,
+                                               float* __restrict__ hi, __nv_bfloat16* __restrict__ h16,
+                                               __nv_bfloat16* __restrict__ l16, int64_t ld, int vec_in,
+                                               int relu_mode) {
+  const int64_t gpr = ld / 8;
+  const int64_t total = R * gpr;
+  const int64_t stride = (int64_t)gridDim.x * blockDim.x;
+  for (int64_t i = (int64_t)blockIdx.x * blockDim.x + threadIdx.x; i < total; i += stride) {
+    const int64_t r = i / gpr, c = (i - r * gpr) * 8;
+    float v[8];
+    if (vec_in && c + 7 < C) {
+      const float4 t0 = *reinterpret_cast<const float4*>(x + r * C + c);
+      const float4 t1 = *reinterpret_cast<const float4*>(x + r * C + c + 4);
+      v[0] = t0.x; v[1] = t0.y; v[2] = t0.z; v[3] = t0.w;
+      v[4] = t1.x; v[5] = t1.y; v[6] = t1.z; v[7] = t1.w;
+    } else {
+#pragma unroll
+      for (int k = 0; k < 8; ++k) v[k] = (c + k < C) ? x[r * C + c + k] : 0.f;
+    }
+    if (relu_mode) {
+#pragma unroll
+      for (int k = 0; k < 8; ++k) v[k] = v[k] < 0.f ? 0.f : v[k];
+    }
+    float h[8];
+    union { __nv_bfloat162 b[4]; uint4 u; } ph, pl;
+#pragma unroll
+    for (int k = 0; k < 8; ++k) h[k] = to_tf32(v[k]);
+#pragma unroll
+    for (int k = 0; k < 4; ++k) {
+      ph.b[k] = __floats2bfloat162_rn(v[2 * k], v[2 * k + 1]);
+      pl.b[k] = __floats2bfloat162_rn(v[2 * k] - h[2 * k], v[2 * k + 1] - h[2 * k + 1]);
+    }
+    float* hp = hi + r * ld + c;
+    *reinterpret_cast<float4*>(hp) = make_float4(h[0], h[1], h[2], h[3]);
+    *reinterpret_cast<float4*>(hp + 4) = make_float4(h[4], h[5], h[6], h[7]);
+    *reinterpret_cast<uint4*>(h16 + r * ld + c) = ph.u;
+    *reinterpret_cast<uint4*>(l16 + r * ld + c) = pl.u;
+  }
+}
+
+struct SplitArgs {
+  const float* x; int64_t R, C; float* hi; __nv_bfloat16* h16; __nv_bfloat16* l16; int64_t ld;
+  int vec_in, relu_mode;
+};
+
+}
+}
```
